# hackmad/pbrt-v3-rs

Hardware: AMD Instinct MI355X
Metric: Mrays/s (higher is better)
Workload: dtype f32

## Files before the change

### include/pbrt_hip.h

```cpp
#ifndef PBRT_HIP_H
#define PBRT_HIP_H

#include <stddef.h>
#include <stdint.h>

#ifdef __cplusplus
extern "C" {
#endif

typedef struct PbrtHipScene PbrtHipScene;

enum {
    PBRT_HIP_OK = 0,
    PBRT_HIP_ERR_INVALID_ARG = -1,
    PBRT_HIP_ERR_STATE = -2,
    PBRT_HIP_ERR_DEVICE = -3,
    PBRT_HIP_ERR_NO_DEVICE = -4,
    PBRT_HIP_ERR_UNSUPPORTED = -5,
    PBRT_HIP_ERR_OOM = -6
};

typedef struct PbrtHipRay {
    float o[3];
    float t_max;
// ... 89 lines not shown
int pbrt_hip_add_texture_checkerboard3d(PbrtHipScene*, uint32_t tex1, uint32_t tex2, const float m[16], uint32_t* out_texture);
enum { PBRT_HIP_PARAM_KD = 0, PBRT_HIP_PARAM_KS = 1, PBRT_HIP_PARAM_KR = 2, PBRT_HIP_PARAM_KT = 3, PBRT_HIP_PARAM_OPACITY = 4, PBRT_HIP_PARAM_AMOUNT = 5, PBRT_HIP_PARAM_ETA = 6,
       PBRT_HIP_PARAM_K = 7, PBRT_HIP_PARAM_REFLECT = 8, PBRT_HIP_PARAM_TRANSMIT = 9 };
int pbrt_hip_set_material_texture(PbrtHipScene*, uint32_t material, int param, uint32_t texture);
int pbrt_hip_set_material_float_texture(PbrtHipScene*, uint32_t material, int fparam, uint32_t texture);
int pbrt_hip_set_material_bump(PbrtHipScene*, uint32_t material, uint32_t texture);
int pbrt_hip_add_material_matte_tex(PbrtHipScene*, uint32_t kd_texture, float sigma_degrees, uint32_t* out_material);
int pbrt_hip_texture_eval_batch(PbrtHipScene*, uint32_t texture, uint64_t n, const float* contexts , float* out_rgb );
int pbrt_hip_texture_eval_batch_nodiff(PbrtHipScene*, uint32_t texture, uint64_t n, const float* contexts , float* out_rgb );
int pbrt_hip_mipmap_levels(PbrtHipScene*, uint32_t mipmap, int* out_levels, int* out_width_height );
int pbrt_hip_mipmap_level_texels(PbrtHipScene*, uint32_t mipmap, int level, float* out_rgb);


int pbrt_hip_add_light_infinite(PbrtHipScene*, const float L_rgb[3], const float light_to_world[16],
                                const float world_to_light[16]);
int pbrt_hip_add_light_infinite_map(PbrtHipScene*, const float L[3], int width, int height, const float* rgb, const float light_to_world[16], const float world_to_light[16]);
int pbrt_hip_add_light_projection(PbrtHipScene*, const float I_rgb[3], const float light_to_world[16], const float world_to_light[16], float fov_deg,
                                  int width, int height, const float* rgb);
int pbrt_hip_add_light_goniometric(PbrtHipScene*, const float I_rgb[3], const float light_to_world[16], const float world_to_light[16],
                                   int width, int height, const float* rgb);
int pbrt_hip_add_light_distant(PbrtHipScene*, const float L_rgb[3], const float w_light_world[3]);
int pbrt_hip_add_light_point(PbrtHipScene*, const float I_rgb[3], const float p_world[3]);
int pbrt_hip_add_light_spot(PbrtHipScene*, const float I_rgb[3], const float light_to_world[16], const float world_to_light[16],
                            float cos_total_width, float cos_falloff_start);
int pbrt_hip_add_light_diffuse_area(PbrtHipScene*, const float L_rgb[3], int two_sided, uint32_t n_tris,
                                    uint32_t* out_first_id);

int pbrt_hip_set_camera_perspective(PbrtHipScene*, const float raster_to_camera[16], const float camera_to_world[16],
                                    float lens_radius, float focal_distance, float shutter_open, float shutter_close);
int pbrt_hip_set_camera_orthographic(PbrtHipScene*, const float raster_to_camera[16], const float camera_to_world[16],
                                     float lens_radius, float focal_distance, float shutter_open, float shutter_close);
int pbrt_hip_set_camera_environment(PbrtHipScene*, const float camera_to_world[16], int xres, int yres, float shutter_open, float shutter_close);

int pbrt_hip_set_film(PbrtHipScene*, int xres, int yres, const int cropped_pixel_bounds[4],
                      const float filter_radius[2], const float filter_table_16x16[256], float scale,
                      float max_sample_luminance);

int pbrt_hip_set_sampler(PbrtHipScene*, int kind, uint32_t samples_per_pixel, const int sample_bounds[4],
                         int sample_at_pixel_center);

int pbrt_hip_set_sobol_tables(PbrtHipScene*, const uint32_t* sobol_matrices32, size_t n32,
                              const uint64_t* vdc_matrices, const uint64_t* vdc_matrices_inv, size_t n_vdc_each);

int pbrt_hip_build_accel(PbrtHipScene*, int split_method, int max_prims_in_node);

int pbrt_hip_build_accel_device(PbrtHipScene*, int split_method, int max_prims_in_node);

int pbrt_hip_world_bound(const PbrtHipScene*, float out_bounds[6]);

int pbrt_hip_accel_stats(const PbrtHipScene*, uint64_t out[8]);
int pbrt_hip_accel_copy(PbrtHipScene*, void* out_nodes, uint64_t node_capacity, void* out_leaf_records, uint64_t record_capacity);


int pbrt_hip_intersect_batch(PbrtHipScene*, const PbrtHipRay* rays, PbrtHipHit* hits, uint64_t n);
int pbrt_hip_occluded_batch(PbrtHipScene*, const PbrtHipRay* rays, uint8_t* out_occluded, uint64_t n);

int pbrt_hip_intersect_batch_device(PbrtHipScene*, const void* d_rays, void* d_hits, uint64_t n, float* kernel_ms);
int pbrt_hip_occluded_batch_device(PbrtHipScene*, const void* d_rays, void* d_occluded, uint64_t n, float* kernel_ms);

int pbrt_hip_set_traversal_counting(PbrtHipScene*, int on);
int pbrt_hip_get_traversal_counts(PbrtHipScene*, uint64_t out[8]);

int pbrt_hip_render_path(PbrtHipScene*, int max_depth, float rr_threshold, int light_strategy,
                         const int pixel_bounds[4], int tile_size, int tile_part, int tile_parts,
                         float* out_xyz, float* out_weight, PbrtHipStats* out_stats);

int pbrt_hip_render_whitted(PbrtHipScene*, int max_depth, const int pixel_bounds[4], int tile_size, int tile_part, int tile_parts,
                            float* out_xyz, float* out_weight, PbrtHipStats* out_stats);

int pbrt_hip_set_sample_record_budget(PbrtHipScene*, uint64_t bytes);
int pbrt_hip_get_render_footprint(PbrtHipScene*, uint64_t out[8]);

int pbrt_hip_tile_buffer_floats(PbrtHipScene*, int tile_size, int tile_part, int tile_parts, uint64_t* out_floats);
int pbrt_hip_render_path_tiles_device(PbrtHipScene*, int max_depth, float rr_threshold, int light_strategy,
                                      const int pixel_bounds[4], int tile_size, int tile_part, int tile_parts,
                                      void* d_tile_buffer, PbrtHipStats* out_stats);
int pbrt_hip_merge_tiles_device(PbrtHipScene*, int tile_size, int tile_parts, const void* const* d_tile_buffers,
                                float* out_xyz, float* out_weight);

int pbrt_hip_film_to_rgb(const PbrtHipScene*, const float* xyz, const float* weight, float* out_rgb);

int pbrt_hip_generate_camera_rays(PbrtHipScene*, const int pixel_bounds[4], uint32_t sample_index,
                                  PbrtHipRay* out_rays, float* out_pfilm_xy);

#ifdef __cplusplus
}
#endif
#endif
```

### pbrt-v3-rs_amd/csrc/api.hip

```cpp
#include "host_math.h"
#include "scene_host.h"
#include "traverse.h"
#include "texture.h"
#include <algorithm>
#include <cstdio>
#include <cstdlib>
#include <mutex>

static std::string g_last_error;
static std::mutex g_err_mu;

namespace phost {

int set_err(PbrtHipScene* s, int code, const std::string& msg) {
    if (s) s->err = msg;
    else { std::lock_guard<std::mutex> g(g_err_mu); g_last_error = msg; }
    return code;
}
int hip_fail(PbrtHipScene* s, hipError_t e, const char* what) {
    std::string m = std::string(what) + ": " + hipGetErrorString(e);
    (void)hipGetLastError();
    return set_err(s, e == hipErrorOutOfMemory ? PBRT_HIP_ERR_OOM : PBRT_HIP_ERR_DEVICE, m);
}
int ensure_buf(PbrtHipScene* s, DevBuf& b, size_t bytes) {
    if (b.bytes >= bytes && b.p) return PBRT_HIP_OK;
    if (b.p) { PH_CHECK(s, hipFree(b.p)); b.p = nullptr; b.bytes = 0; }
    if (bytes == 0) bytes = 16;
    PH_CHECK(s, hipMalloc(&b.p, bytes));
    b.bytes = bytes;
    if (bytes <= 4096) PH_CHECK(s, hipMemset(b.p, 0, bytes));
    return PBRT_HIP_OK;
}

template <class T> static int upload_vec(PbrtHipScene* s, const std::vector<T>& v, const T** out) {
    *out = nullptr;
    if (v.empty()) return PBRT_HIP_OK;
    void* d = nullptr;
    PH_CHECK(s, hipMalloc(&d, v.size() * sizeof(T)));
    s->owned.push_back(d);
    PH_CHECK(s, hipMemcpyAsync(d, v.data(), v.size() * sizeof(T), hipMemcpyHostToDevice, s->stream));
    *out = reinterpret_cast<const T*>(d);
    return PBRT_HIP_OK;
}

void free_tree_dev(PbrtHipScene* s) {
    if (s->tree_dev_nodes) (void)hipFree(s->tree_dev_nodes);
    if (s->tree_dev_tris) (void)hipFree(s->tree_dev_tris);
    s->tree_dev_nodes = s->tree_dev_tris = nullptr; s->tree_dev_n_tris = 0;
}

static void free_owned(PbrtHipScene* s) {
    for (void* p : s->owned) (void)hipFree(p);
    s->owned.clear();
    s->uploaded = false;
    s->light_strategy_uploaded = -1;
}

static hm::HaltonTables& halton_tables() {
    static hm::HaltonTables t;
    static std::once_flag once;
    std::call_once(once, []() { t.build(); });
    return t;
}

__global__ void patch_inst_records_kernel(TriRec* tris, uint32_t n_top, const InstRec* inst, float* extra) {
    const uint32_t i = blockIdx.x * blockDim.x + threadIdx.x;
    if (i >= n_top) return;
    uint32_t f = tris[i].flags & ~PH_TRI_NEXT_INST;
    if (!(f & PH_TRI_LAST) && i + 1u < n_top && (tris[i + 1u].flags & PH_TRI_INSTANCE)) f |= PH_TRI_NEXT_INST;
    if (f & PH_TRI_INSTANCE) {
        const InstRec& I = inst[tris[i].prim];
        const bool general = !(I.w2i[12] == 0.0f && I.w2i[13] == 0.0f && I.w2i[14] == 0.0f && I.w2i[15] == 1.0f);
        for (int k = 0; k < 3; k++) { tris[i].p0[k] = I.lo[k]; tris[i].p1[k] = I.hi[k]; }
        tris[i].p2[0] = __uint_as_float(I.root_ref); tris[i].p2[1] = __uint_as_float(I.flags | (general ? PH_INST_GENERAL : 0u)); tris[i].p2[2] = 0.0f;
        for (int k = 0; k < 12; k++) extra[12 * (size_t)i + k] = I.w2i[k];
    }
    tris[i].flags = f;
}
__global__ void patch_leaf_refs_kernel(Node64* nodes, uint32_t n_nodes, const TriRec* tris, uint32_t n_top) {
    const uint32_t i = blockIdx.x * blockDim.x + threadIdx.x;
    if (i >= n_nodes) return;
    uint32_t c[2] = {nodes[i].c0, nodes[i].c1};
    for (int k = 0; k < 2; k++)
        if ((c[k] & PH_LEAF_BIT) && c[k] < PH_NEED_POP) {
            const uint32_t t = c[k] & ~(PH_LEAF_BIT | PH_LEAF_INST_HINT);
            c[k] = PH_LEAF_BIT | t | ((t < n_top && (tris[t].flags & PH_TRI_INSTANCE)) ? PH_LEAF_INST_HINT : 0u);
        }
    nodes[i].c0 = c[0]; nodes[i].c1 = c[1];
}

int upload_scene(PbrtHipScene* s) {
    if (s->uploaded) return PBRT_HIP_OK;
    free_owned(s);
    DeviceScene& d = s->ds;
    std::memset(&d, 0, sizeof(d));
    int rc;
    if (s->tree_dev_tris) { d.nodes = reinterpret_cast<const Node64*>(s->tree_dev_nodes); d.tris = reinterpret_cast<const TriRec*>(s->tree_dev_tris); }
    else {
        if ((rc = upload_vec(s, s->bvh.nodes, &d.nodes))) return rc;
        if ((rc = upload_vec(s, s->bvh.tris, &d.tris))) return rc;
    }
    d.root_ref = s->bvh.root_ref;
    d.n_tris = (uint32_t)(s->idx.size() / 3);
    for (int k = 0; k < 3; k++) { d.root_lo[k] = s->bvh.root_lo[k]; d.root_hi[k] = s->bvh.root_hi[k]; d.world_center[k] = s->world_center[k]; }
    d.world_radius = s->world_radius;
    if ((rc = upload_vec(s, s->P, &d.P))) return rc;
    if (s->any_n && (rc = upload_vec(s, s->N, &d.N))) return rc;
    if (s->any_s && (rc = upload_vec(s, s->S, &d.S))) return rc;
    if (s->any_uv && (rc = upload_vec(s, s->UV, &d.UV))) return rc;
    if ((rc = upload_vec(s, s->idx, &d.idx))) return rc;
    if ((rc = upload_vec(s, s->tri_mesh, &d.tri_mesh))) return rc;
    if ((rc = upload_vec(s, s->tri_flags, &d.tri_flags))) return rc;
    if (s->emission_only.empty()) { if ((rc = upload_vec(s, s->meshes, &d.meshes))) return rc; }
    else {
        std::vector<MeshRec> meshes(s->meshes);
        for (MeshRec& m : meshes) if (m.first_light <= -2) m.first_light = (int32_t)(s->lights.size() + (size_t)(-2 - m.first_light));
        if ((rc = upload_vec(s, meshes, &d.meshes))) return rc;
    }
    {
        for (MaterialRec& m : s->materials) {
            uint32_t cols = m.amount_tex1 ? 1u : 0u; bool hdr = m.bump_tex1 != 0u || m.sigma_tex1 != 0u;
            for (uint32_t k = 0; k < m.n_lobes; k++) {
                s->lobes[m.lobe_base + k].slot0 = cols;
                const LobeRec& l = s->lobes[m.lobe_base + k];
                if (l.has_pre == PH_PRE_RT) { cols += 1u; hdr = true; }
                else cols += (l.r_tex1 || (l.has_pre == PH_PRE_OPACITY && l.kind != PH_LK_SPEC_T) ? 1u : 0u) + (l.t_tex1 || (l.has_pre == PH_PRE_OPACITY && l.kind == PH_LK_SPEC_T) || l.has_pre == PH_PRE_PASSTHROUGH ? 1u : 0u) +
                        (l.eta_tex1 ? 1u : 0u) + (l.k_tex1 ? 1u : 0u);
                if (l.sigma_tex1 || l.ax_tex1 || l.ay_tex1 || l.alt || l.has_pre == PH_PRE_RAW_TEST) hdr = true;
            }
            if (m.sigma_tex1 || hdr) cols = std::max(cols, 2u);
            if (m.index_tex1) cols = std::max(cols, 3u);
            if (m.rt_mode) hdr = true;
            m.tex_cols = std::min<uint32_t>(cols, PH_HIT_COLS); m.tex_hdr = hdr ? 1u : 0u;
        }
        s->alpha_lean = s->alpha_textures;
        for (const MeshRec& m : s->meshes)
            for (uint32_t t1 : {m.alpha_tex1, m.shadow_alpha_tex1})
                if (t1)
                    for (const TexOp& op : s->textures[t1 - 1u].prog)
                        if (!(op.op == PH_TOP_CONST || op.op == PH_TOP_MUL || op.op == PH_TOP_MIX || (op.op == PH_TOP_IMAGE && op.mapping == 0u))) s->alpha_lean = false;
        s->simple_textures = true;
        for (const PbrtHipScene::TextureHost& t : s->textures)
            for (const TexOp& op : t.prog)
                if (!(op.op == PH_TOP_CONST || op.op == PH_TOP_MUL || op.op == PH_TOP_MIX || (op.op == PH_TOP_IMAGE && op.mapping == 0u))) s->simple_textures = false;
    }
    if ((rc = upload_vec(s, s->materials, &d.materials))) return rc;
    if ((rc = upload_vec(s, s->lobes, &d.lobes))) return rc;
    {
        const uint32_t kMaxTex = 500u, kMaxPlain = 500u;
        std::vector<uint16_t> key(std::max<size_t>(s->materials.size(), 1), 0);
        uint32_t n_tex = 0, n_plain = 0;
        for (const MaterialRec& m : s->materials) if (!m.none && (m.textured || m.bump_tex1)) n_tex++;
        const uint32_t T = std::min(n_tex, kMaxTex);
        uint32_t jt = 0, jp = 0;
        for (size_t i = 0; i < s->materials.size(); i++) {
            const MaterialRec& m = s->materials[i];
            if (!m.none && (m.textured || m.bump_tex1)) key[i] = (uint16_t)std::min(jt++, kMaxTex - 1u);
            else { key[i] = (uint16_t)(T + std::min(jp++, kMaxPlain - 1u)); n_plain++; }
        }
        const uint32_t U = std::min(n_plain, kMaxPlain);
        if ((rc = upload_vec(s, key, &d.mat_key))) return rc;
        d.ms_tex_keys = T; d.ms_key_emit = T + U; d.ms_key_idle = T + U + 1u;
    }
    if (!s->textures.empty() || !s->mipmaps.empty()) {
        std::vector<TexRec> recs; std::vector<TexOp> ops;
        for (const PbrtHipScene::TextureHost& t : s->textures) {
            recs.push_back(TexRec{(uint32_t)ops.size(), (uint32_t)t.prog.size()});
            ops.insert(ops.end(), t.prog.begin(), t.prog.end());
        }
        std::vector<float> lut(PH_EWA_LUT_SIZE);
        for (int i = 0; i < PH_EWA_LUT_SIZE; i++) {
            const float r2 = (float)i / (float)(PH_EWA_LUT_SIZE - 1);
            lut[(size_t)i] = std::exp(-2.0f * r2) - std::exp(-2.0f);
        }
        if ((rc = upload_vec(s, recs, &d.textures))) return rc;
        if ((rc = upload_vec(s, ops, &d.tex_ops))) return rc;
        if ((rc = upload_vec(s, s->mipmaps, &d.mipmaps))) return rc;
        if ((rc = upload_vec(s, s->texels, &d.texels))) return rc;
        if ((rc = upload_vec(s, lut, &d.ewa_lut))) return rc;
    }
    if (s->emission_only.empty()) { if ((rc = upload_vec(s, s->lights, &d.lights))) return rc; }
    else {
        std::vector<LightRec> all(s->lights);
        all.insert(all.end(), s->emission_only.begin(), s->emission_only.end());
        if ((rc = upload_vec(s, all, &d.lights))) return rc;
    }
    if ((rc = upload_vec(s, s->light_dist, &d.light_dist))) return rc;
    d.n_lights = (uint32_t)s->lights.size();
    if ((rc = upload_vec(s, s->infinite_lights, &d.infinite_lights))) return rc;
    d.n_infinite = (uint32_t)s->infinite_lights.size();
    if ((rc = upload_vec(s, s->inst_recs, &d.instances))) return rc;
    if ((rc = upload_vec(s, s->quadrics, &d.quadrics))) return rc;
    d.n_instances = (uint32_t)s->inst_recs.size();
    if (!s->inst_recs.empty() && !s->top_items.empty() && d.tris) {
        const uint32_t n_top = (uint32_t)s->top_items.size();
        const uint32_t n_nodes = (uint32_t)(s->tree_dev_tris ? s->bvh.interior_nodes : s->bvh.nodes.size());
        void* extra = nullptr;
        PH_CHECK(s, hipMalloc(&extra, (size_t)n_top * 48)); s->owned.push_back(extra);
        hipLaunchKernelGGL(patch_inst_records_kernel, dim3((n_top + 255u) / 256u), dim3(256), 0, s->stream, const_cast<TriRec*>(d.tris), n_top, d.instances, static_cast<float*>(extra));
        if (n_nodes) hipLaunchKernelGGL(patch_leaf_refs_kernel, dim3((n_nodes + 255u) / 256u), dim3(256), 0, s->stream, const_cast<Node64*>(d.nodes), n_nodes, d.tris, n_top);
        PH_CHECK(s, hipGetLastError());
        d.inst_extra = static_cast<const float*>(extra);
    }
    hm::HaltonTables& ht = halton_tables();
    if ((rc = upload_vec(s, ht.perms, &d.halton_perms))) return rc;
    if ((rc = upload_vec(s, ht.primes, &d.primes))) return rc;
    if ((rc = upload_vec(s, ht.prime_sums, &d.prime_sums))) return rc;
    if ((rc = upload_vec(s, ht.magic, &d.prime_magic))) return rc;
    if ((rc = upload_vec(s, s->sobol32, &d.sobol32))) return rc;
    if ((rc = upload_vec(s, s->vdc, &d.vdc))) return rc;
    if ((rc = upload_vec(s, s->vdc_inv, &d.vdc_inv))) return rc;
    {
        void* dself = nullptr;
        PH_CHECK(s, hipMalloc(&dself, sizeof(DeviceScene)));
        s->owned.push_back(dself);
        d.self = reinterpret_cast<const DeviceScene*>(dself);
        PH_CHECK(s, hipMemcpyAsync(dself, &d, sizeof(DeviceScene), hipMemcpyHostToDevice, s->stream));
    }
    PH_CHECK(s, hipStreamSynchronize(s->stream));
    s->uploaded = true;
    return PBRT_HIP_OK;
}

int upload_light_distribution(PbrtHipScene* s, int light_strategy) {
    const size_t n = s->lights.size();
    int strat = (n == 1) ? 0 : light_strategy;
    if (s->light_strategy_uploaded == strat) return PBRT_HIP_OK;
    std::vector<float> f(n, 1.0f), cdf;
    float func_int = 0.0f;
    if (strat == 1) {
        const float wr = s->world_radius;
        for (size_t i = 0; i < n; i++) {
            const LightRec& l = s->lights[i];
            float p[3];
            for (int c = 0; c < 3; c++) {
                switch (l.type) {
                case PH_L_INFINITE: {
                    if (l.map_mip1) { float t[3]; hmip_lookup_triangle(s, s->mipmaps[l.map_mip1 - 1u], 0.5f, 0.5f, 0.5f, t); p[c] = hm::kPi * wr * wr * t[c]; break; }
                    float tx = l.L[c];
                    float v = tx * (1.0f - 0.0f) * (1.0f - 0.0f) + tx * (1.0f - 0.0f) * 0.0f + tx * 0.0f * (1.0f - 0.0f) + tx * 0.0f * 0.0f;
                    p[c] = hm::kPi * wr * wr * v;
                    break;
                }
                case PH_L_DISTANT: p[c] = l.L[c] * hm::kPi * wr * wr; break;
                case PH_L_POINT: p[c] = (hm::kPi * 4.0f) * l.L[c]; break;
                case PH_L_PROJECTION: case PH_L_GONIO: {
                    float t[3] = {1.0f, 1.0f, 1.0f};
                    if (l.map_mip1) hmip_lookup_triangle(s, s->mipmaps[l.map_mip1 - 1u], 0.5f, 0.5f, 0.5f, t);
                    p[c] = l.type == PH_L_PROJECTION ? t[c] * l.L[c] * (2.0f * hm::kPi) * (1.0f - l.cos_total_width) : (hm::kPi * 4.0f) * l.L[c] * t[c];
                    break;
                }
                case PH_L_SPOT: p[c] = l.L[c] * (2.0f * hm::kPi) * (1.0f - 0.5f * (l.cos_falloff_start + l.cos_total_width)); break;
                default: p[c] = (l.two_sided ? 2.0f : 1.0f) * l.L[c] * l.area * hm::kPi; break;
                }
            }
            f[i] = 0.212671f * p[0] + 0.715160f * p[1] + 0.072169f * p[2];
        }
    }
    if (n) hm::distribution1d(f, cdf, func_int);
    int rc;
    if ((rc = ensure_buf(s, s->d_ld_func, std::max<size_t>(n, 1) * 4))) return rc;
    if ((rc = ensure_buf(s, s->d_ld_cdf, (n + 1) * 4))) return rc;
    if (n) {
        PH_CHECK(s, hipMemcpy(s->d_ld_func.p, f.data(), n * 4, hipMemcpyHostToDevice));
        PH_CHECK(s, hipMemcpy(s->d_ld_cdf.p, cdf.data(), (n + 1) * 4, hipMemcpyHostToDevice));
    }
    s->ds.ld_func = (const float*)s->d_ld_func.p; s->ds.ld_cdf = (const float*)s->d_ld_cdf.p; s->ds.ld_func_int = func_int;
    s->light_strategy_uploaded = strat;
    return PBRT_HIP_OK;
}

int ensure_traversal_workspace(PbrtHipScene* s) {
    if (!s->trav_blocks) {
        hipDeviceProp_t prop;
        PH_CHECK(s, hipGetDeviceProperties(&prop, s->device));
        int per_cu = 0;
        PH_CHECK(s, hipOccupancyMaxActiveBlocksPerMultiprocessor(&per_cu, ph::traverse_kernel<ph::ShapeFlat, ph::TRAV_MIXED>, PH_TRAV_BLOCK, 0));
        per_cu = std::max(std::min(per_cu, ph::ShapeFlat::wpe), 1);
        s->trav_blocks = (uint32_t)(prop.multiProcessorCount * per_cu);
    }
    const uint32_t total_threads = s->trav_blocks * PH_TRAV_BLOCK;
    int rc;
    if ((rc = ensure_buf(s, s->d_counter, 64))) return rc;
    if ((rc = ensure_buf(s, s->d_error, 64))) return rc;
    if ((rc = ensure_buf(s, s->d_counts, 64 + 36 * 8))) return rc;
    const bool inst = !s->inst_recs.empty();
    if ((rc = ensure_buf(s, s->d_spill, (size_t)(ph::trav_stack_cap(inst) - ph::TravShapes::spill_lds_depth(inst)) * total_threads * sizeof(uint2)))) return rc;
    return PBRT_HIP_OK;
}

template <class Shape>
static void launch_traverse_shape(PbrtHipScene* s, int mode, uint32_t blocks, const ph::TravParams& p) {
    const dim3 g(blocks), b(PH_TRAV_BLOCK);
    if (mode == ph::TRAV_MIXED) hipLaunchKernelGGL((ph::traverse_kernel<Shape, ph::TRAV_MIXED>), g, b, 0, s->stream, s->ds, p);
    else if (mode == ph::TRAV_ANY) hipLaunchKernelGGL((ph::traverse_kernel<Shape, ph::TRAV_ANY>), g, b, 0, s->stream, s->ds, p);
    else hipLaunchKernelGGL((ph::traverse_kernel<Shape, ph::TRAV_CLOSEST>), g, b, 0, s->stream, s->ds, p);
}
template <class... S>
static void dispatch_traverse_shape(ph::ShapeTable<S...>, int shape, PbrtHipScene* s, int mode, uint32_t blocks, const ph::TravParams& p) {
    static constexpr void (*launchers[])(PbrtHipScene*, int, uint32_t, const ph::TravParams&) = {&launch_traverse_shape<S>...};
    launchers[shape](s, mode, blocks, p);
}

// ... 868 lines not shown
    if (out_first_id) *out_first_id = (uint32_t)s->lights.size();
    for (uint32_t i = 0; i < n_tris; i++) {
        LightRec l{}; l.type = PH_L_AREA; l.two_sided = two_sided ? 1 : 0; l.prim = 0xFFFFFFFFu;
        for (int c = 0; c < 3; c++) l.L[c] = L[c];
        s->lights.push_back(l);
    }
    s->uploaded = false;
    return PBRT_HIP_OK;
    });
}

int pbrt_hip_set_camera_perspective(PbrtHipScene* s, const float r2c[16], const float c2w[16], float lens_radius, float focal_distance,
                                    float shutter_open, float shutter_close) {
    return ph_guard(s, "pbrt_hip_set_camera_perspective", [&]() -> int {
    if (!s || !r2c || !c2w) return set_err(s, PBRT_HIP_ERR_INVALID_ARG, "set_camera_perspective: null argument");
    std::memcpy(s->cam.r2c, r2c, 64); std::memcpy(s->cam.c2w, c2w, 64);
    s->cam.lens_radius = lens_radius; s->cam.focal_distance = focal_distance;
    s->cam.shutter_open = shutter_open; s->cam.shutter_close = shutter_close;
    {
        auto pt = [&](float x, float y, float out[3]) {
            const float* m = r2c;
            const float xp = m[0] * x + m[1] * y + m[2] * 0.0f + m[3], yp = m[4] * x + m[5] * y + m[6] * 0.0f + m[7];
            const float zp = m[8] * x + m[9] * y + m[10] * 0.0f + m[11], wp = m[12] * x + m[13] * y + m[14] * 0.0f + m[15];
            if (wp == 1.0f) { out[0] = xp; out[1] = yp; out[2] = zp; }
            else { const float inv = 1.0f / wp; out[0] = inv * xp; out[1] = inv * yp; out[2] = inv * zp; }
        };
        float p0[3], px[3], py[3];
        pt(0.0f, 0.0f, p0); pt(1.0f, 0.0f, px); pt(0.0f, 1.0f, py);
        for (int k = 0; k < 3; k++) { s->cam.dx_camera[k] = px[k] - p0[k]; s->cam.dy_camera[k] = py[k] - p0[k]; }
    }
    s->cam.kind = PH_CAM_PERSPECTIVE;
    s->have_camera = true;
    return PBRT_HIP_OK;
    });
}
int pbrt_hip_set_camera_orthographic(PbrtHipScene* s, const float r2c[16], const float c2w[16], float lens_radius, float focal_distance,
                                     float shutter_open, float shutter_close) {
    return ph_guard(s, "pbrt_hip_set_camera_orthographic", [&]() -> int {
    const int rc = pbrt_hip_set_camera_perspective(s, r2c, c2w, lens_radius, focal_distance, shutter_open, shutter_close);
    if (rc != PBRT_HIP_OK) return rc;
    const float* m = r2c;
    const float vx[3] = {1.0f, 0.0f, 0.0f}, vy[3] = {0.0f, 1.0f, 0.0f};
    for (int k = 0; k < 3; k++) {
        s->cam.dx_camera[k] = m[4 * k] * vx[0] + m[4 * k + 1] * vx[1] + m[4 * k + 2] * vx[2];
        s->cam.dy_camera[k] = m[4 * k] * vy[0] + m[4 * k + 1] * vy[1] + m[4 * k + 2] * vy[2];
    }
    s->cam.kind = PH_CAM_ORTHOGRAPHIC;
    return PBRT_HIP_OK;
    });
}

int pbrt_hip_set_camera_environment(PbrtHipScene* s, const float c2w[16], int xres, int yres, float shutter_open, float shutter_close) {
    return ph_guard(s, "pbrt_hip_set_camera_environment", [&]() -> int {
    if (!s || !c2w) return set_err(s, PBRT_HIP_ERR_INVALID_ARG, "set_camera_environment: null argument");
    if (xres <= 0 || yres <= 0) return set_err(s, PBRT_HIP_ERR_INVALID_ARG, "set_camera_environment: the film's full resolution must be positive");
    s->cam = CameraRec{};
    for (int k = 0; k < 4; k++) s->cam.r2c[5 * k] = 1.0f;
    std::memcpy(s->cam.c2w, c2w, 64);
    s->cam.focal_distance = 1e6f; s->cam.shutter_open = shutter_open; s->cam.shutter_close = shutter_close;
    s->cam.full_res[0] = (float)xres; s->cam.full_res[1] = (float)yres;
    s->cam.kind = PH_CAM_ENVIRONMENT;
    s->have_camera = true;
    return PBRT_HIP_OK;
    });
}

int pbrt_hip_set_film(PbrtHipScene* s, int xres, int yres, const int crop[4], const float radius[2], const float table[256], float scale,
                      float max_lum) {
    return ph_guard(s, "pbrt_hip_set_film", [&]() -> int {
    if (!s || !crop || !radius || !table) return set_err(s, PBRT_HIP_ERR_INVALID_ARG, "set_film: null argument");
    if (!(radius[0] > 0.0f) || !(radius[1] > 0.0f)) return set_err(s, PBRT_HIP_ERR_INVALID_ARG, "set_film: filter radius must be positive");
    FilmRec& f = s->film;
    f.xres = xres; f.yres = yres;
    for (int i = 0; i < 4; i++) f.crop[i] = crop[i];
    f.radius[0] = radius[0]; f.radius[1] = radius[1];
    f.inv_radius[0] = 1.0f / radius[0]; f.inv_radius[1] = 1.0f / radius[1];
    f.scale = scale; f.max_lum = max_lum;
    std::memcpy(f.table, table, sizeof(f.table));
    s->have_film = true;
    return PBRT_HIP_OK;
    });
}

static void ext_gcd(uint64_t a, uint64_t b, int64_t& x, int64_t& y) {
    if (b == 0) { x = 1; y = 0; return; }
    int64_t d = (int64_t)(a / b), xp, yp;
    ext_gcd(b, a % b, xp, yp);
    x = yp; y = xp - (d * yp);
}
static uint64_t mult_inverse(int64_t a, int64_t n) {
    int64_t x, y;
    ext_gcd((uint64_t)a, (uint64_t)n, x, y);
    int64_t r = x - (x / n) * n;
    return (uint64_t)(r < 0 ? r + n : r);
}

int pbrt_hip_set_sampler(PbrtHipScene* s, int kind, uint32_t spp, const int sb[4], int at_center) {
    return ph_guard(s, "pbrt_hip_set_sampler", [&]() -> int {
    if (!s || !sb) return set_err(s, PBRT_HIP_ERR_INVALID_ARG, "set_sampler: null argument");
    if (kind != 0 && kind != 1) return set_err(s, PBRT_HIP_ERR_UNSUPPORTED, "set_sampler: only halton (0) and sobol (1) are GPU-friendly (SURVEY §8a-S)");
    if (spp == 0) return set_err(s, PBRT_HIP_ERR_INVALID_ARG, "set_sampler: spp must be > 0");
    SamplerRec& r = s->sampler;
    std::memset(&r, 0, sizeof(r));
    r.kind = kind; r.spp = spp; r.at_center = at_center ? 1 : 0;
    for (int i = 0; i < 4; i++) r.bounds[i] = sb[i];
    if (kind == 0) {
        int res[2] = {sb[2] - sb[0], sb[3] - sb[1]};
        for (int i = 0; i < 2; i++) {
            uint64_t base = i == 0 ? 2 : 3, scale = 1, e = 0;
            while ((int)scale < std::min(res[i], 128)) { scale *= base; e++; }
            r.base_scales[i] = (uint32_t)scale; r.base_exponents[i] = (uint32_t)e;
        }
        r.sample_stride = r.base_scales[0] * r.base_scales[1];
        r.mult_inverse[0] = (uint32_t)mult_inverse(r.base_scales[1], r.base_scales[0]);
        r.mult_inverse[1] = (uint32_t)mult_inverse(r.base_scales[0], r.base_scales[1]);
        if (((uint64_t)spp + 1) * r.sample_stride >= (1ull << 32))
            return set_err(s, PBRT_HIP_ERR_UNSUPPORTED, "set_sampler: halton index exceeds 32 bits at this spp/resolution");
    } else {
        auto pow2_up = [](uint32_t v) { v--; v |= v >> 1; v |= v >> 2; v |= v >> 4; v |= v >> 8; v |= v >> 16; return v + 1; };
        if (spp & (spp - 1)) r.spp = pow2_up(spp);
        int ext = std::max(sb[2] - sb[0], sb[3] - sb[1]);
        r.resolution = (int)pow2_up((uint32_t)std::max(ext, 1));
        int lg = 0; for (uint32_t v = (uint32_t)r.resolution; v >>= 1;) lg++;
        r.log2_resolution = lg;
    }
    s->have_sampler = true;
    return PBRT_HIP_OK;
    });
}

int pbrt_hip_set_sobol_tables(PbrtHipScene* s, const uint32_t* m32, size_t n32, const uint64_t* vdc, const uint64_t* vdc_inv, size_t n_each) {
    return ph_guard(s, "pbrt_hip_set_sobol_tables", [&]() -> int {
    if (!s || !m32 || !vdc || !vdc_inv) return set_err(s, PBRT_HIP_ERR_INVALID_ARG, "set_sobol_tables: null argument");
    if (n32 == 0 || n32 % 52 || n_each % 52) return set_err(s, PBRT_HIP_ERR_INVALID_ARG, "set_sobol_tables: table lengths must be non-zero multiples of 52");
    s->sobol32.assign(m32, m32 + n32); s->vdc.assign(vdc, vdc + n_each); s->vdc_inv.assign(vdc_inv, vdc_inv + n_each);
    s->uploaded = false;
    return PBRT_HIP_OK;
    });
}

int pbrt_hip_build_accel(PbrtHipScene* s, int split_method, int max_prims_in_node) {
    return ph_guard(s, "pbrt_hip_build_accel", [&]() -> int {
    if (!s) return PBRT_HIP_ERR_INVALID_ARG;
    if (split_method == 2) return set_err(s, PBRT_HIP_ERR_UNSUPPORTED, "build_accel: splitmethod 'middle' panics in the reference (quirk B6, sah.rs:67-76)");
    if (!s->quadrics.empty()) {
        if (s->build_on_device) return set_err(s, PBRT_HIP_ERR_UNSUPPORTED, "build_accel_device: a scene with quadric shapes is built on the host (pbrt_hip_build_accel)");
        if (!s->objects.empty() || !s->instances.empty()) return set_err(s, PBRT_HIP_ERR_UNSUPPORTED, "build_accel: quadric shapes together with object definitions or instances are not supported");
        s->prim_quadric.resize(s->idx.size() / 3, 0u);
    }
    for (size_t i = 0; i < s->lights.size(); i++)
        if (s->lights[i].type == PH_L_AREA && s->lights[i].prim == 0xFFFFFFFFu)
            return set_err(s, PBRT_HIP_ERR_STATE, "build_accel: area light " + std::to_string(i) + " was never attached to a mesh (pbrt_hip_add_mesh first_area_light_id)");
    {
        std::vector<uint64_t> sigs;
        for (MaterialRec& m : s->materials) {
            uint64_t sig = 1;
            for (uint32_t k = 0; k < m.n_lobes; k++) sig = sig * 8 + (s->lobes[m.lobe_base + k].kind + 1);
            size_t c = 0;
            while (c < sigs.size() && sigs[c] != sig) c++;
            if (c == sigs.size()) sigs.push_back(sig);
            m.sort_class = (uint32_t)std::min<size_t>(c, 6);
            if (m.none) m.sort_class = 7u;
        }
    }
    if (s->tree_dev_tris) { PH_CHECK(s, hipSetDevice(s->device)); free_tree_dev(s); }
    std::vector<uint32_t> build_flags(s->tri_flags);
    for (size_t t = 0; t < build_flags.size(); t++) {
        const uint32_t mat = s->meshes[s->tri_mesh[t]].material;
        build_flags[t] |= (s->materials[mat].sort_class << PH_TRI_CLASS_SHIFT) | (std::min<uint32_t>(mat, 0xFFFu) << PH_TRI_MAT_SHIFT);
    }
    phost::BuildInput in;
    in.P = s->P.data(); in.idx = s->idx.data(); in.n_tris = s->idx.size() / 3; in.tri_flags = build_flags.data(); in.tri_mesh = s->tri_mesh.data();
    if (!s->quadrics.empty()) { in.prim_quadric = s->prim_quadric.data(); in.quad_bounds = s->quadric_bounds.data(); }
    auto fail = [&](int brc) {
        if (brc == -2) return set_err(s, PBRT_HIP_ERR_INVALID_ARG, "build_accel: the reference's HLBVH build asserts on this input (hlbvh.rs:338/356/418)");
        return set_err(s, PBRT_HIP_ERR_INVALID_ARG, "build_accel: bad arguments");
    };
    s->inst_recs.clear();
    if (s->objects.empty()) {
        int brc;
        if (s->build_on_device) {
            PH_CHECK(s, hipSetDevice(s->device));
            std::string e;
            if (split_method == 1) brc = phost::build_hlbvh_device(in, max_prims_in_node, s->stream, s->bvh, e);
            else {
                brc = phost::build_sah_device(in, max_prims_in_node, s->stream, s->bvh, e, &s->tree_dev_nodes, &s->tree_dev_tris);
                if (brc == 0 && s->tree_dev_tris) s->tree_dev_n_tris = in.n_tris;
            }
            if (brc == -1) return set_err(s, PBRT_HIP_ERR_DEVICE, "build_accel_device: " + e);
        } else brc = phost::build_bvh(in, split_method, max_prims_in_node, 0, s->bvh);
        if (brc != 0) return fail(brc);
    } else {
        if (s->open_object >= 0) return set_err(s, PBRT_HIP_ERR_STATE, "build_accel: an object definition is still open (missing ObjectEnd)");
        std::vector<uint32_t> tri0(s->objects.size()), tri1(s->objects.size()), inst_object(s->instances.size());
        std::vector<float> inst_i2w(16 * s->instances.size());
        for (size_t k = 0; k < s->objects.size(); k++) { tri0[k] = s->objects[k].tri0; tri1[k] = s->objects[k].tri1; }
        for (size_t k = 0; k < s->instances.size(); k++) { inst_object[k] = s->instances[k].object; std::memcpy(&inst_i2w[16 * k], s->instances[k].i2w, 64); }
        const phost::InstancedScene isc{tri0.data(), tri1.data(), tri0.size(), inst_object.data(), inst_i2w.data(), inst_object.size(), s->top_items.data(), s->top_items.size()};
// ... 204 lines not shown
```

### pbrt-v3-rs_amd/csrc/host_math.h

```cpp
#pragma once
#include <cmath>
#include <cstdint>
#include <cstring>
#include <vector>

namespace hm {

constexpr float kPi = 3.14159265358979323846f;
constexpr float kInf = __builtin_huge_valf();

inline float fabs_p(float n) { return n < 0.0f ? -n : n; }
inline float clampf(float x, float lo, float hi) { return x < lo ? lo : (x > hi ? hi : x); }
inline float to_radians(float d) { return d * (kPi / 180.0f); }

struct V3 { float x, y, z; };
inline V3 sub(V3 a, V3 b) { return {a.x - b.x, a.y - b.y, a.z - b.z}; }
inline V3 add(V3 a, V3 b) { return {a.x + b.x, a.y + b.y, a.z + b.z}; }
inline V3 mulf(V3 a, float f) { return {a.x * f, a.y * f, a.z * f}; }
inline V3 divf(V3 a, float f) { float inv = 1.0f / f; return {inv * a.x, inv * a.y, inv * a.z}; }
inline V3 cross(V3 a, V3 b) { return {(a.y * b.z) - (a.z * b.y), (a.z * b.x) - (a.x * b.z), (a.x * b.y) - (a.y * b.x)}; }
inline float len2(V3 a) { return a.x * a.x + a.y * a.y + a.z * a.z; }
inline float len(V3 a) { return std::sqrt(len2(a)); }
inline V3 normalize(V3 a) { return divf(a, len(a)); }
inline void coordinate_system(V3 v1, V3& v2, V3& v3) {
    if (std::fabs(v1.x) > std::fabs(v1.y)) v2 = divf({-v1.z, 0.0f, v1.x}, std::sqrt(v1.x * v1.x + v1.z * v1.z));
    else v2 = divf({0.0f, v1.z, -v1.y}, std::sqrt(v1.y * v1.y + v1.z * v1.z));
    v3 = cross(v1, v2);
}
inline V3 ld(const float* p) { return {p[0], p[1], p[2]}; }

struct Pcg32 {
    uint64_t state = 0x853c49e6748fea9bULL, inc = 0xda3e39cb94b95bdbULL;
    uint32_t next() {
        uint64_t old = state;
        state = old * 0x5851f42d4c957f2dULL + inc;
        uint32_t xs = (uint32_t)(((old >> 18) ^ old) >> 27), rot = (uint32_t)(old >> 59);
        return (xs >> rot) | (xs << ((~rot + 1) & 31));
    }
    uint32_t bounded(uint32_t lo, uint32_t hi) {
        uint32_t b = hi - lo, threshold = (~b + 1) % b;
        for (;;) { uint32_t r = next(); if (r >= threshold) return lo + r % b; }
    }
};

inline float radical_inverse(uint32_t base, uint64_t a) {
    if (base == 2) {
        uint64_t n = a;
        n = ((n >> 1) & 0x5555555555555555ULL) | ((n & 0x5555555555555555ULL) << 1);
        n = ((n >> 2) & 0x3333333333333333ULL) | ((n & 0x3333333333333333ULL) << 2);
        n = ((n >> 4) & 0x0f0f0f0f0f0f0f0fULL) | ((n & 0x0f0f0f0f0f0f0f0fULL) << 4);
        n = ((n >> 8) & 0x00ff00ff00ff00ffULL) | ((n & 0x00ff00ff00ff00ffULL) << 8);
        n = ((n >> 16) & 0x0000ffff0000ffffULL) | ((n & 0x0000ffff0000ffffULL) << 16);
        n = (n >> 32) | (n << 32);
        return (float)n * 0x1.0p-64f;
    }
    const float inv_base = 1.0f / (float)base;
    uint64_t reversed = 0; float inv_base_n = 1.0f;
    while (a != 0) {
        const uint64_t next = a / base, digit = a - next * base;
        reversed = reversed * base + digit;
        inv_base_n *= inv_base;
        a = next;
    }
    const float v = (float)reversed * inv_base_n;
    return v < 0x1.fffffep-1f ? v : 0x1.fffffep-1f;
}

struct HaltonTables {
    std::vector<uint32_t> primes, prime_sums;
    std::vector<uint16_t> perms;
    std::vector<uint64_t> magic;
    void build() {
        primes.clear(); prime_sums.clear();
        for (uint32_t c = 2; primes.size() < 1000; c++) {
            bool is_p = true;
            for (uint32_t q : primes) { if (q * q > c) break; if (c % q == 0) { is_p = false; break; } }
            if (is_p) primes.push_back(c);
        }
        uint32_t total = 0;
        magic.clear();
        for (uint32_t p : primes) { prime_sums.push_back(total); total += p; magic.push_back((uint64_t)(((unsigned __int128)1 << 64) / p) + 1); }
        perms.assign(total, 0);
        Pcg32 rng; size_t at = 0;
        for (uint32_t p : primes) {
            for (uint32_t j = 0; j < p; j++) perms[at + j] = (uint16_t)j;
            for (uint32_t j = 0; j < p; j++) {
                uint32_t other = j + rng.bounded(0, p - j);
                uint16_t t = perms[at + j]; perms[at + j] = perms[at + other]; perms[at + other] = t;
            }
            at += p;
        }
    }
};

inline void distribution1d(const std::vector<float>& f, std::vector<float>& cdf, float& func_int) {
    size_t n = f.size();
    cdf.assign(n + 1, 0.0f);
    for (size_t i = 1; i < n + 1; i++) cdf[i] = cdf[i - 1] + f[i - 1] / (float)n;
    func_int = cdf[n];
    if (func_int == 0.0f) for (size_t i = 1; i < n + 1; i++) cdf[i] = (float)i / (float)n;
    else for (size_t i = 1; i < n + 1; i++) cdf[i] /= func_int;
}

struct M4 { float m[4][4]; };
inline M4 m4_identity() { M4 r; for (int i = 0; i < 4; i++) for (int j = 0; j < 4; j++) r.m[i][j] = i == j ? 1.0f : 0.0f; return r; }
inline M4 m4_mul(const M4& a, const M4& b) {
    M4 r;
    for (int i = 0; i < 4; i++)
        for (int j = 0; j < 4; j++)
            r.m[i][j] = a.m[i][0] * b.m[0][j] + a.m[i][1] * b.m[1][j] + a.m[i][2] * b.m[2][j] + a.m[i][3] * b.m[3][j];
    return r;
}
inline M4 m4_transpose(const M4& a) { M4 r; for (int i = 0; i < 4; i++) for (int j = 0; j < 4; j++) r.m[i][j] = a.m[j][i]; return r; }
M4 m4_inverse(const M4& a);

}
```

### pbrt-v3-rs_amd/csrc/pt_device.h

```cpp
#pragma once
#include "dmath.h"
#include "scene_types.h"
#include "traverse.h"

namespace ph {

struct f2 { float x, y; };
PH_DEV f2 mk2(float x, float y) { f2 r; r.x = x; r.y = y; return r; }

PH_DEV float radical_inverse_2(uint64_t a) {
    uint64_t r = ((uint64_t)__brev((uint32_t)a) << 32) | (uint64_t)__brev((uint32_t)(a >> 32));
    return __ull2float_rn(r) * 0x1.0p-64f;
}
PH_DEV float radical_inverse_base(uint32_t base, uint32_t a) {
    const float inv_base = ph_div(1.0f, (float)base);
    uint64_t reversed = 0;
    float inv_base_n = 1.0f;
    while (a != 0) {
        uint32_t next = a / base, digit = a - next * base;
        reversed = reversed * base + digit;
        inv_base_n *= inv_base;
        a = next;
    }
    return pminf(__ull2float_rn(reversed) * inv_base_n, kOneMinusEps);
}
PH_DEV float scrambled_radical_inverse(uint32_t base, uint64_t magic, uint32_t a, const uint16_t* __restrict__ perm) {
    const float inv_base = ph_div(1.0f, (float)base);
    uint64_t reversed = 0;
    float inv_base_n = 1.0f;
    while (a != 0) {
        uint32_t next = (uint32_t)__umul64hi((uint64_t)a, magic), digit = a - next * base;
        reversed = reversed * base + perm[digit];
        inv_base_n *= inv_base;
        a = next;
    }
    return pminf(inv_base_n * (__ull2float_rn(reversed) + ph_div(inv_base * (float)perm[0], 1.0f - inv_base)), kOneMinusEps);
}
PH_DEV uint32_t inverse_radical_inverse(uint32_t base, uint32_t inverse, uint32_t n_digits) {
    uint32_t index = 0;
    for (uint32_t i = 0; i < n_digits; i++) { uint32_t digit = inverse % base; inverse /= base; index = index * base + digit; }
    return index;
}
PH_DEV int rem_i(int a, int b) { int r = a - (a / b) * b; return r < 0 ? r + b : r; }

PH_DEV uint32_t halton_pixel_offset(const SamplerRec& sp, int px, int py) {
    uint64_t off = 0;
    if (sp.sample_stride > 1) {
        const int pm[2] = {rem_i(px, 128), rem_i(py, 128)};
        for (int i = 0; i < 2; i++) {
            uint64_t dim_offset = inverse_radical_inverse(i == 0 ? 2u : 3u, (uint32_t)pm[i], sp.base_exponents[i]);
            off += dim_offset * (uint64_t)(sp.sample_stride / sp.base_scales[i]) * (uint64_t)sp.mult_inverse[i];
        }
        off %= sp.sample_stride;
    }
    return (uint32_t)off;
}
#define PH_LDS_DIMS 54
#define PH_LDS_PERMS 6081
struct HaltonLds {
    uint8_t perms[PH_LDS_PERMS + 2];
    uint32_t primes[PH_LDS_DIMS], sums[PH_LDS_DIMS];
    uint64_t magic[PH_LDS_DIMS];
};
PH_DEV void halton_lds_fill(HaltonLds* l, const DeviceScene& sc) {
    for (uint32_t i = threadIdx.x; i < PH_LDS_PERMS; i += blockDim.x) l->perms[i] = (uint8_t)sc.halton_perms[i];
    for (uint32_t i = threadIdx.x; i < PH_LDS_DIMS; i += blockDim.x) { l->primes[i] = sc.primes[i]; l->sums[i] = sc.prime_sums[i]; l->magic[i] = sc.prime_magic[i]; }
}
PH_DEV float scrambled_radical_inverse_lds(const HaltonLds* l, uint32_t dim, uint32_t a) {
    const uint32_t base = l->primes[dim];
    const uint64_t magic = l->magic[dim];
    const uint8_t* perm = l->perms + l->sums[dim];
    const float inv_base = ph_div(1.0f, (float)base);
    uint64_t reversed = 0;
    float inv_base_n = 1.0f;
    while (a != 0) {
        uint32_t next = (uint32_t)__umul64hi((uint64_t)a, magic), digit = a - next * base;
        reversed = reversed * base + perm[digit];
        inv_base_n *= inv_base;
        a = next;
    }
    return pminf(inv_base_n * (__ull2float_rn(reversed) + ph_div(inv_base * (float)perm[0], 1.0f - inv_base)), kOneMinusEps);
}
PH_DEV float halton_sample(const DeviceScene& sc, const SamplerRec& sp, uint32_t index, uint32_t dim, const HaltonLds* lds = nullptr) {
    if (sp.at_center && (dim == 0 || dim == 1)) return 0.5f;
    if (dim == 0) return radical_inverse_2((uint64_t)(index >> sp.base_exponents[0]));
    if (dim == 1) return radical_inverse_base(3u, index / sp.base_scales[1]);
    if (lds && dim < PH_LDS_DIMS) return scrambled_radical_inverse_lds(lds, dim, index);
    return scrambled_radical_inverse(sc.primes[dim], sc.prime_magic[dim], index, sc.halton_perms + sc.prime_sums[dim]);
}

PH_DEV uint64_t sobol_interval_to_index(const DeviceScene& sc, uint32_t m, uint64_t frame, int px, int py) {
    if (m == 0) return 0;
    const uint32_t m2 = m << 1;
    uint64_t index = frame << m2;
    uint64_t delta = 0;
    for (int c = 0; frame != 0; frame >>= 1, c++)
        if (frame & 1) delta ^= sc.vdc[(size_t)(m - 1) * 52 + c];
    uint64_t b = ((((uint64_t)(uint32_t)px) << m) | ((uint64_t)(uint32_t)py)) ^ delta;
    for (int c = 0; b != 0; b >>= 1, c++)
        if (b & 1) index ^= sc.vdc_inv[(size_t)(m - 1) * 52 + c];
    return index;
}
PH_DEV float sobol_sample(const DeviceScene& sc, const SamplerRec& sp, uint64_t a, uint32_t dim, int px, int py) {
    uint32_t v = 0;
    for (size_t i = (size_t)dim * 52; a != 0; a >>= 1, i++)
        if (a & 1) v ^= sc.sobol32[i];
    float s = pminf((float)v * 0x1.0p-32f, kOneMinusEps);
    if (dim == 0 || dim == 1) {
        s = s * (float)sp.resolution + (float)sp.bounds[dim];
        s = pclampf(s - (float)(dim == 0 ? px : py), 0.0f, kOneMinusEps);
    }
    return s;
}

struct SamplerCursor {
    uint64_t index;
    uint32_t dim;
    int px, py;
    const HaltonLds* lds;
};
PH_DEV float sampler_dim(const DeviceScene& sc, const SamplerRec& sp, const SamplerCursor& c, uint32_t dim) {
    return sp.kind == 0 ? halton_sample(sc, sp, (uint32_t)c.index, dim, c.lds) : sobol_sample(sc, sp, c.index, dim, c.px, c.py);
}
PH_DEV float get_1d(const DeviceScene& sc, const SamplerRec& sp, SamplerCursor& c) {
    float p = sampler_dim(sc, sp, c, c.dim);
    c.dim += 1;
    return p;
}
PH_DEV f2 get_2d(const DeviceScene& sc, const SamplerRec& sp, SamplerCursor& c) {
    if (c.dim + 1 >= 5 && c.dim < 5) c.dim = 5;
    f2 p = mk2(sampler_dim(sc, sp, c, c.dim), sampler_dim(sc, sp, c, c.dim + 1));
    c.dim += 2;
    return p;
}

PH_DEV f2 concentric_sample_disk(f2 u) {
    f2 uo = mk2(2.0f * u.x - 1.0f, 2.0f * u.y - 1.0f);
    if (uo.x == 0.0f && uo.y == 0.0f) return mk2(0.0f, 0.0f);
    float r, theta;
    if (pabs(uo.x) > pabs(uo.y)) { r = uo.x; theta = kPiOver4 * ph_div(uo.y, uo.x); }
    else { r = uo.y; theta = kPiOver2 - kPiOver4 * ph_div(uo.x, uo.y); }
    float sn, cs;
    d_sincos(theta, sn, cs);
    return mk2(r * cs, r * sn);
}
PH_DEV f3 cosine_sample_hemisphere(f2 u) {
    f2 d = concentric_sample_disk(u);
    float z = ph_sqrt(pmaxf(0.0f, 1.0f - d.x * d.x - d.y * d.y));
    return mk3(d.x, d.y, z);
}
PH_DEV f2 uniform_sample_triangle(f2 u) { float su0 = ph_sqrt(u.x); return mk2(1.0f - su0, u.y * su0); }
PH_DEV float power_heuristic1(float fp, float gp) {
    float f = 1.0f * fp, g = 1.0f * gp;
    return ph_div(f * f, f * f + g * g);
}
PH_DEV uint32_t find_interval_cdf(const float* cdf, uint32_t size, float u) {
    uint32_t first = 0, len = size;
    while (len > 0) {
        uint32_t half = len >> 1, middle = first + half;
        if (cdf[middle] <= u) { first = middle + 1; len -= half + 1; }
        else len = half;
    }
    if (first == 0) return 0;
    uint32_t v = first - 1, hi = size - 2;
    return v > hi ? hi : v;
}

__device__ __noinline__ void environment_camera_dir(float px, float py, float xres, float yres, f3* out) {
    const float theta = ph_div(kPi * py, yres), phi = ph_div(kTwoPi * px, xres);
    const float st = d_sin(theta);
    *out = mk3(st * d_cos(phi), d_cos(theta), st * d_sin(phi));
}
PH_DEV void generate_camera_ray(const CameraRec& cam, f2 p_film, float time_s, f2 lens_s, RayIn& out) {
    const float* m = cam.r2c;
    float xp = m[0] * p_film.x + m[1] * p_film.y + m[2] * 0.0f + m[3];
    float yp = m[4] * p_film.x + m[5] * p_film.y + m[6] * 0.0f + m[7];
    float zp = m[8] * p_film.x + m[9] * p_film.y + m[10] * 0.0f + m[11];
    float wp = m[12] * p_film.x + m[13] * p_film.y + m[14] * 0.0f + m[15];
    f3 p_camera = (wp == 1.0f) ? mk3(xp, yp, zp) : mk3(xp, yp, zp) / wp;
    f3 o = mk3(0.0f, 0.0f, 0.0f), d = normalize(p_camera);
    if (cam.kind == PH_CAM_ORTHOGRAPHIC) { o = p_camera; d = mk3(0.0f, 0.0f, 1.0f); }
    if (cam.kind == PH_CAM_ENVIRONMENT) environment_camera_dir(p_film.x, p_film.y, cam.full_res[0], cam.full_res[1], &d);
    const float time = (1.0f - time_s) * cam.shutter_open + time_s * cam.shutter_close;
    if (cam.lens_radius > 0.0f) {
        f2 cd = concentric_sample_disk(lens_s);
        f2 p_lens = mk2(cam.lens_radius * cd.x, cam.lens_radius * cd.y);
        float ft = ph_div(cam.focal_distance, d.z);
        f3 p_focus = o + d * ft;
        o = mk3(p_lens.x, p_lens.y, 0.0f);
        d = normalize(p_focus - o);
    }
    const float* c = cam.c2w;
    float ox = (c[0] * o.x + c[1] * o.y) + (c[2] * o.z + c[3]);
    float oy = (c[4] * o.x + c[5] * o.y) + (c[6] * o.z + c[7]);
    float oz = (c[8] * o.x + c[9] * o.y) + (c[10] * o.z + c[11]);
    float ow = (c[12] * o.x + c[13] * o.y) + (c[14] * o.z + c[15]);
    float xs = pabs(c[0] * o.x) + pabs(c[1] * o.y) + pabs(c[2] * o.z) + pabs(c[3]);
    float ys = pabs(c[4] * o.x) + pabs(c[5] * o.y) + pabs(c[6] * o.z) + pabs(c[7]);
    float zs = pabs(c[8] * o.x) + pabs(c[9] * o.y) + pabs(c[10] * o.z) + pabs(c[11]);
    f3 o_err = kGamma3 * mk3(xs, ys, zs);
    f3 ow3 = (ow == 1.0f) ? mk3(ox, oy, oz) : mk3(ox, oy, oz) / ow;
    f3 dw = mk3(c[0] * d.x + c[1] * d.y + c[2] * d.z, c[4] * d.x + c[5] * d.y + c[6] * d.z, c[8] * d.x + c[9] * d.y + c[10] * d.z);
    float l2 = length_squared(dw), t_max = kInf;
    if (l2 > 0.0f) {
        float dt = ph_div(dot(vabs(dw), o_err), l2);
// ... 393 lines not shown
```

### pbrt-v3-rs_amd/csrc/scene_host.h

```cpp
#pragma once
#include "../../include/pbrt_hip.h"
#include "band_plan.h"
#include "bvh_build.h"
#include "guard.h"
#include "scene_types.h"
#include <hip/hip_runtime.h>
namespace ph { struct TravParams; }
#include <string>
#include <vector>

struct DevBuf {
    void* p = nullptr;
    size_t bytes = 0;
};

struct SceneHostState {
    std::vector<float> P, N, S, UV;
    bool any_n = false, any_s = false, any_uv = false;
    std::vector<uint32_t> idx, tri_mesh, tri_flags;
    std::vector<MeshRec> meshes;
    std::vector<QuadricRec> quadrics;
    std::vector<float> quadric_bounds;
    std::vector<uint32_t> prim_quadric;
    std::vector<MaterialRec> materials;
    std::vector<LobeRec> lobes;
    struct TextureHost { std::vector<TexOp> prog; int stack_need = 1; };
    std::vector<TextureHost> textures;
    std::vector<MipRec> mipmaps;
    std::vector<Texel> texels;
    struct MaterialParams { int lobe[4] = {-1, -1, -1, -1}; int field[4] = {0, 0, 0, 0}; int lobe2[4] = {-1, -1, -1, -1}; int field2[4] = {0, 0, 0, 0}; bool has_pre = false; float pre[3] = {1, 1, 1}; int rough_lobe = -1, rough_lobe2 = -1; bool rough_remap = false;
                            int made_as = 0;   float raw_k[4][3] = {{0, 0, 0}, {0, 0, 0}, {0, 0, 0}, {0, 0, 0}}; float raw_eta = 1.5f, raw_ur = 0, raw_vr = 0;
                            bool raw_remap = false, rebuilt = false; int mix_n1 = 0; };
    std::vector<MaterialParams> material_params;
    bool alpha_textures = false;
    bool alpha_lean = false;
    bool bump_materials = false;
    bool textured_materials = false;
    bool has_none_material = false;
    bool general_materials = false;
    bool simple_textures = false;
    std::vector<LightRec> lights;
    uint32_t sphere_lights = 0;
    std::vector<LightRec> emission_only;
    std::vector<uint32_t> infinite_lights;
    std::vector<float> light_dist;
    struct ObjectHost { uint32_t tri0 = 0, tri1 = 0; };
    struct InstanceHost { uint32_t object; float i2w[16], w2i[16]; };
    std::vector<ObjectHost> objects;
    std::vector<InstanceHost> instances;
    std::vector<uint32_t> top_items;
    int open_object = -1;
    std::vector<InstRec> inst_recs;
    CameraRec cam{};
    FilmRec film{};
    SamplerRec sampler{};
    bool have_camera = false, have_film = false, have_sampler = false, built = false;
    std::vector<uint32_t> sobol32;
    std::vector<uint64_t> vdc, vdc_inv;

    phost::BuildOutput bvh;
    float world_center[3] = {0, 0, 0}, world_radius = 1.0f;
};

struct MultiDevice;

struct PbrtHipScene : SceneHostState {
    int device = 0;
    hipStream_t stream = nullptr;
    std::string err;
    bool build_on_device = false;
    MultiDevice* multi = nullptr;

    DeviceScene ds{};
    std::vector<void*> owned;
    void* tree_dev_nodes = nullptr; void* tree_dev_tris = nullptr; size_t tree_dev_n_tris = 0;
    bool uploaded = false;
    int light_strategy_uploaded = -1;
    DevBuf d_ld_func, d_ld_cdf;

    DevBuf d_counter, d_spill, d_error, d_rays_tmp, d_out_tmp;
    uint32_t trav_blocks = 0;
    bool count_traversal = false;
    DevBuf d_counts;
    hipEvent_t ev0 = nullptr, ev1 = nullptr;

    struct Wavefront* wf = nullptr;
    struct WhittedWorkspace* wh = nullptr;

    uint64_t record_budget = 0;
    uint64_t footprint[8] = {0, 0, 0, 0, 0, 0, 0, 0};
};

namespace phost {
int set_err(PbrtHipScene* s, int code, const std::string& msg);
int hip_fail(PbrtHipScene* s, hipError_t e, const char* what);
int ensure_buf(PbrtHipScene* s, DevBuf& b, size_t bytes);
int upload_scene(PbrtHipScene* s);
void projection_light_setup(float fov_deg, float aspect, float out_proj[16], float out_screen[4], float* out_cos_total_width);
void hmip_lookup_triangle(const PbrtHipScene* s, const MipRec& m, float u, float v, float width, float out[3]);
int upload_light_distribution(PbrtHipScene* s, int light_strategy);
int launch_traverse(PbrtHipScene* s, bool anyhit, const void* d_rays, void* d_out, uint32_t n, float* kernel_ms);
void launch_traverse_kernel(PbrtHipScene* s, int mode, uint32_t blocks, const ph::TravParams& p);
int ensure_traversal_workspace(PbrtHipScene* s);
void free_wavefront(PbrtHipScene* s);
int build_hlbvh_device(const BuildInput& in, int max_prims_in_node, hipStream_t stream, BuildOutput& out, std::string& err, const ForestSpec* forest = nullptr,
                       std::vector<ForestTreeOut>* trees_out = nullptr);
int build_sah_device(const BuildInput& in, int max_prims_in_node, hipStream_t stream, BuildOutput& out, std::string& err, void** keep_nodes = nullptr, void** keep_tris = nullptr,
                     const ForestSpec* forest = nullptr, std::vector<ForestTreeOut>* trees_out = nullptr);
void free_tree_dev(PbrtHipScene* s);
int uber_rebuild_for_opacity(PbrtHipScene* s, uint32_t material);
int glass_rebuild_for_roughness(PbrtHipScene* s, uint32_t material);
int translucent_rebuild_rt(PbrtHipScene* s, uint32_t material);
#define PH_MAX_TILE_PARTS 64
int check_render_args(PbrtHipScene* s, int max_depth, int light_strategy, const int* pixel_bounds, int tile_size, int part, int parts);
size_t tile_buffer_floats_for(const PbrtHipScene* s, int tile_size, int part, int parts);
int render_tiles(PbrtHipScene* s, int max_depth, float rr_threshold, int light_strategy, const int pixel_bounds[4], int tile_size, int part, int parts, void* d_tile_buffer,
                 PbrtHipStats* out_stats);
int merge_tiles(PbrtHipScene* s, int tile_size, int parts, const void* const* d_bufs, float* out_xyz, float* out_weight);
DevBuf& tile_buffer_of(PbrtHipScene* s);
int merge_own_tiles(PbrtHipScene* s, int tile_size, int tile_part, int tile_parts, float* out_xyz, float* out_weight);
struct SampleRecords { uint32_t n_px; const int2* px_xy; float4* rec_L; float* rec_py; uint8_t* px_rounded; SampleBand band; uint32_t band_px; std::vector<SampleBand> bands; };
int samples_begin(PbrtHipScene* s, int tile_size, int part, int parts, SampleRecords* out);
int samples_plan_bands(PbrtHipScene* s, SampleRecords* out, size_t chunk_held, size_t chunk_per_path);
int samples_alloc(PbrtHipScene* s, SampleRecords* out);
int samples_band(PbrtHipScene* s, const SampleRecords& r, size_t band, SampleRecords* out);
int samples_to_tiles(PbrtHipScene* s, const SampleRecords& r, void* d_tile_buffer);
size_t path_chunk_bytes_per_path(bool general_materials, bool textured_materials);
void free_whitted(PbrtHipScene* s);
size_t whitted_chunk_bytes_per_sample(uint32_t n_frames);
int spatial_voxels_touched(PbrtHipScene* s, std::vector<uint8_t>& touched, uint64_t* count);
int render_path_multi(PbrtHipScene* s, int max_depth, float rr_threshold, int light_strategy, const int pixel_bounds[4], int tile_size, int tile_part, int tile_parts,
                      float* out_xyz, float* out_weight, PbrtHipStats* out_stats);
void free_multi(PbrtHipScene* s);
}

#define PH_CHECK(s, call)                                              \
    do {                                                               \
        hipError_t e__ = (call);                                       \
        if (e__ != hipSuccess) return phost::hip_fail((s), e__, #call); \
    } while (0)
```

### pbrt-v3-rs_amd/csrc/scene_types.h

```cpp
#pragma once
#include <stdint.h>

#define PH_LEAF_BIT 0x80000000u
#define PH_INVALID_REF 0xFFFFFFFFu
#define PH_NEED_POP 0xFFFFFFFEu
#define PH_LEAF_INST_HINT 0x40000000u
struct alignas(64) Node64 {
    float x0[2], y0[2], z0[2];
    float x1[2], y1[2], z1[2];
    uint32_t c0, c1;
    uint32_t axis;
    uint32_t pad;
};

#define PH_TRI_LAST 1u
#define PH_TRI_BOGUS 2u
#define PH_TRI_ALPHA0 4u
#define PH_TRI_SALPHA0 8u
#define PH_TRI_CLASS_SHIFT 8
#define PH_TRI_MAT_SHIFT 11
#define PH_TRI_KEY_MASK 0x7FFFu
#define PH_TRI_ALPHATEX 32u
#define PH_TRI_NEXT_INST 64u
#define PH_TRI_INSTANCE 16u
// ... 85 lines not shown
    uint32_t refl_tex1, trans_tex1;
    float refl_c[3], trans_c[3];
    uint32_t index_tex1;
    uint32_t tex_cols;
    uint32_t tex_hdr;
};
#define PH_HIT_COLS 6
struct TexOut { float ns[3]; uint32_t bumped; float dpdu_s[3]; uint32_t lambert; float col[PH_HIT_COLS][4]; };
#define PH_HIT_LOBES 8

enum { PH_TOP_CONST = 0, PH_TOP_IMAGE = 1, PH_TOP_MUL = 2, PH_TOP_MIX = 3, PH_TOP_CHECKER = 4 , PH_TOP_UV = 5,
       PH_TOP_BILERP = 6 , PH_TOP_DOTS = 7 , PH_TOP_FBM = 8, PH_TOP_WRINKLED = 9, PH_TOP_WINDY = 10, PH_TOP_MARBLE = 11,
       PH_TOP_CHECKER3D = 12  };
#define PH_TEX_STACK 6
struct TexOp {
    uint32_t op;
    uint32_t mip;
    float c[3];
    float su, sv, du, dv;
    uint32_t octaves;
    float omega, scale, variation;
    float m[16];
    uint32_t mapping;
    uint32_t pad_[3];
};
struct TexRec { uint32_t first_op, n_ops; };
struct Texel { float r, g, b, pad; };
#define PH_MIP_MAX_LEVELS 16
struct MipRec {
    uint32_t n_levels, filtering , wrap , is_float;
    float max_anisotropy;
    uint32_t pad[3];
    uint32_t level_off[PH_MIP_MAX_LEVELS];
    uint32_t level_w[PH_MIP_MAX_LEVELS], level_h[PH_MIP_MAX_LEVELS];
};
#define PH_EWA_LUT_SIZE 128

enum { PH_L_INFINITE = 0, PH_L_DISTANT = 1, PH_L_POINT = 2, PH_L_AREA = 3, PH_L_SPOT = 4, PH_L_PROJECTION = 5, PH_L_GONIO = 6 };
struct LightRec {
    int32_t type;
    int32_t two_sided;
    uint32_t prim;
    float area;
    float L[3];
    uint32_t map_mip1;
    float v[3];
    uint32_t dist_off;
    float l2w[12];
    float w2l[12];
    float cond_func[4], cond_cdf[6], cond_int[2];
    float marg_func[2], marg_cdf[3], marg_int;
    float cos_total_width, cos_falloff_start;
    uint32_t dw, dh;
    float proj[16];
    float screen[4];
};

enum { PH_CAM_PERSPECTIVE = 0, PH_CAM_ORTHOGRAPHIC = 1, PH_CAM_ENVIRONMENT = 2 };
struct CameraRec {
    float r2c[16];
    float c2w[16];
    float lens_radius, focal_distance, shutter_open, shutter_close;
    float dx_camera[3], dy_camera[3];
    uint32_t kind; float pad[1];
    float full_res[2];
};

struct FilmRec {
    int32_t xres, yres;
    int32_t crop[4];
    float radius[2], inv_radius[2];
    float scale, max_lum;
    float table[256];
};

struct SamplerRec {
    int32_t kind;
    uint32_t spp;
    int32_t bounds[4];
    int32_t at_center;
    uint32_t base_scales[2], base_exponents[2], sample_stride;
    uint32_t mult_inverse[2];
    int32_t resolution, log2_resolution;
};

struct DeviceScene {
    const Node64* nodes;
    const TriRec* tris;
    uint32_t root_ref;
    uint32_t n_tris;
    float root_lo[3], root_hi[3];
    float world_center[3], world_radius;
    const float* P;
    const float* N;
    const float* S;
    const float* UV;
    const uint32_t* idx;
    const uint32_t* tri_mesh;
    const uint32_t* tri_flags;
    const MeshRec* meshes;
    const MaterialRec* materials;
    const LobeRec* lobes;
    const TexRec* textures;
    const TexOp* tex_ops;
    const MipRec* mipmaps;
    const Texel* texels;
    const float* ewa_lut;
    const float* light_dist;
    const DeviceScene* self;
    const LightRec* lights;
    uint32_t n_lights;
    const uint32_t* infinite_lights;
    uint32_t n_infinite;
    const uint16_t* mat_key;
    uint32_t ms_tex_keys, ms_key_emit, ms_key_idle;
    const InstRec* instances;
    const float* inst_extra;
    uint32_t n_instances;
    const float* ld_func;
    const float* ld_cdf;
    float ld_func_int;
    const uint16_t* halton_perms;
    const uint32_t* primes;
    const uint32_t* prime_sums;
    const uint64_t* prime_magic;
    const uint32_t* sobol32;
    const uint64_t* vdc;
    const uint64_t* vdc_inv;
    const QuadricRec* quadrics;
};
```

### pbrt-v3-rs_amd/csrc/wavefront.hip

```cpp
#define PH_OUTLINE_MATH 1
#include "host_math.h"
#include "pt_device.h"
#include "scene_host.h"
#include "spatial.h"
#include "bsdf_general.h"
#include "texture.h"
#include "raysort.h"
#include "phase_clock.h"
#include "matsort.h"
#include "wf_device.h"
#include "chunk_plan.h"
#include <algorithm>
#include <cstdlib>

namespace ph {

enum : uint32_t { F_EXT = 1u, F_PSH = 2u, F_PMIS = 4u, F_SPEC = 8u, F_NODIFF = 16u };

struct IterCounters {
    uint32_t n_cl, n_sh, n_live, head_cl, head_sh, pad[3];
};
struct DevStats { unsigned long long camera_rays, paths_total, paths_zero; };

struct TileInfo {
// ... 271 lines not shown
                    if (!w.occ[idx4.z]) est = est + mks(A4.x, A4.y, A4.z);
                }
                if (flags & F_PMIS) {
                    const float4 F4 = w.s_f2[it & 1][prev];
                    const uint32_t light_num = __float_as_uint(F4.w);
                    const RayIn mr = load_ray(rays_in + idx4.y);
                    const float4* hp = reinterpret_cast<const float4*>(w.hits_cl + idx4.y);
                    const float4 h0 = hp[0];
                    const uint32_t hprim = __float_as_uint(h0.y);
                    const f3 wi = mk3(mr.dx, mr.dy, mr.dz);
                    spec li2 = mks1(0.0f);
                    if (hprim != 0xFFFFFFFFu) {
                        const LightRec& lt = sc.lights[light_num];
                        if (lt.type == PH_L_AREA && lt.prim == hprim) {
                            const float4 h1 = hp[1];
                            MeshRec m;
                            SurfHit lh = make_surface_hit_any(sc, wi, mr.time, __float_as_uint(h1.y), __float_as_uint(h1.z), h0.z, h0.w, h1.x, m);
                            li2 = area_L(lt, lh.n, -wi);
                        }
                    } else li2 = light_le<TEX>(sc, sc.lights[light_num], wi);
                    if (!is_black(li2)) est = est + mks(F4.x, F4.y, F4.z) * li2 * mks1(1.0f) * A4.w / O4.w;
                }
                const spec ldv = mks(O4.x, O4.y, O4.z) * (est / L4.w);
                if (is_black(ldv)) n_paths_zero++;
                L = L + ldv;
                flags &= ~(F_PSH | F_PMIS);
            }
            PHC_END(0);

            if (flags & F_EXT) {
                flags &= ~F_EXT;
                const RayIn ray = load_ray(rays_in + idx4.x);
                const float4* hp = reinterpret_cast<const float4*>(w.hits_cl + idx4.x);
                const float4 h0 = hp[0];
                const uint32_t hprim = __float_as_uint(h0.y);
                const bool found = hprim != 0xFFFFFFFFu;
                const f3 rd = mk3(ray.dx, ray.dy, ray.dz);
                const bool emit = bounces == 0 || (GEN && (flags & F_SPEC));
                if (!found) {
                    if (emit)
                        for (uint32_t k = 0; k < sc.n_infinite; k++) L = L + beta * light_le<TEX>(sc, sc.lights[sc.infinite_lights[k]], rd);
                } else {
                    const float4 h1 = hp[1];
                    MeshRec m;
                    PHC_BEGIN(1);
                    QSurf qs;
                    SurfHit si = QUADRIC ? make_surface_hit_q<QUADRIC>(sc, mk3(ray.ox, ray.oy, ray.oz), rd, ray.time, __float_as_uint(h1.y), __float_as_uint(h1.z), h0.z, h0.w, h1.x, m, &qs)
                                         : make_surface_hit_any(sc, rd, ray.time, __float_as_uint(h1.y), __float_as_uint(h1.z), h0.z, h0.w, h1.x, m);
                    if (emit) {
                        if (m.first_light >= 0) L = L + beta * area_L(sc.lights[(uint32_t)m.first_light + (hprim - m.tri_base)], si.n, -rd);
                        else L = L + beta * mks1(0.0f);
                    }
                    PHC_END(1);
                    bool no_bsdf = sc.materials[m.material].none != 0u;
                    if (TEX && !no_bsdf && sc.materials[m.material].rt_mode) no_bsdf = (w.tex_out[i].bumped & PH_TEXOUT_NULL_BSDF) != 0u;
                    if ((int)bounces < w.max_depth && no_bsdf) {
                        const RayIn re = spawn_ray(si, rd);
                        flags |= F_EXT | F_NODIFF; want_ext = true;
                        stage[0][0][tid] = make_float4(re.ox, re.oy, re.oz, re.t_max);
                        stage[0][1][tid] = make_float4(re.dx, re.dy, re.dz, re.time);
                    } else if ((int)bounces < w.max_depth) {
                        const uint32_t ppix = pid / w.chunk_spp;
                        const int2 xy = w.px_xy[ppix];
                        bool tex_hit = false;
                        if (TEX) {
                            const MaterialRec& mr = sc.materials[m.material];
                            tex_hit = mr.textured != 0u || mr.bump_tex1 != 0u;
                            if (tex_hit && mr.bump_tex1) {
                                const float4* tp = reinterpret_cast<const float4*>(w.tex_out + i);
                                const float4 f0 = tp[0], f1 = tp[1];
                                si.ns = mk3(f0.x, f0.y, f0.z); si.dpdu_s = mk3(f1.x, f1.y, f1.z);
                            }
                        }
                        PHC_BEGIN(2);
                        typename BO::T bsdf = BO::make(sc, si, m.material);
                        if (TEX && tex_hit) {
                            const MaterialRec& mr = sc.materials[m.material];
                            if (mr.textured)
                                BO::apply_textures(bsdf, w.tex_out + i, mr);
                        }
                        PHC_END(2);
                        PHC_BEGIN(3);
                        SamplerCursor cur = cursor_for(sc, w.sp, xy.x, xy.y, w.s0 + (pid - ppix * w.chunk_spp), dim, hl);
#pragma unroll 1
                        for (uint32_t k = 0; k < 8; k++) s_u[k][tid] = sampler_dim(sc, w.sp, cur, dim + k);
                        PHC_END(3);
                        uint32_t c = 0;
                        if (BO::has_non_specular(bsdf)) {
                            n_paths_total++;
                            if (sc.n_lights > 0) {
                                PHC_BEGIN(4);
                                const float sample = s_u[0][tid]; c = 1;
                                const float* ld_func = sc.ld_func; const float* ld_cdf = sc.ld_cdf; float ld_func_int = sc.ld_func_int;
                                if (w.spatial.enabled) {
                                    const int32_t slot = w.spatial.vox_slot[spatial_voxel_of(w.spatial, si.p)];
                                    if (slot >= 0) {
                                        ld_func = w.spatial.pool + (size_t)slot * w.spatial.stride;
                                        ld_cdf = ld_func + sc.n_lights; ld_func_int = ld_cdf[sc.n_lights + 1];
                                    } else ld_func_int = 0.0f;
                                }
                                const uint32_t light_num = (sc.n_lights == 1) ? 0u : find_interval_cdf(ld_cdf, sc.n_lights + 1, sample);
                                pick_pdf = ld_func_int > 0.0f ? ph_div(ld_func[light_num], ld_func_int * (float)sc.n_lights) : 0.0f;
                                PHC_END(4);
                                if (pick_pdf != 0.0f) {
                                    const LightRec& light = sc.lights[light_num];
                                    const f2 u_light = mk2(s_u[1][tid], s_u[2][tid]), u_scatter = mk2(s_u[3][tid], s_u[4][tid]); c = 5;
                                    const bool is_delta = light.type == PH_L_DISTANT || light.type == PH_L_POINT || light.type == PH_L_SPOT || light.type == PH_L_PROJECTION || light.type == PH_L_GONIO;
                                    float w2 = 0.0f, spdf_store = 0.0f;
                                    spec A = mks1(0.0f);
                                    {
                                        PHC_BEGIN(5);
                                        const LiSample ls = light_sample_li<TEX>(sc, light, si, u_light);
                                        PHC_END(5);
                                        PHC_BEGIN(6);
                                        if (ls.valid && ls.pdf > 0.0f && !is_black(ls.value)) {
                                            const spec f = BO::f_ns(bsdf, si.wo, ls.wi) * abs_dot(ls.wi, si.ns);
                                            const float scattering_pdf = BO::pdf_ns(bsdf, si.wo, ls.wi);
                                            if (!is_black(f)) {
                                                const RayIn rs = spawn_ray_to_hit(si, ls.vp, ls.vperr, ls.vn);
                                                stage[2][0][tid] = make_float4(rs.ox, rs.oy, rs.oz, rs.t_max);
                                                stage[2][1][tid] = make_float4(rs.dx, rs.dy, rs.dz, rs.time);
                                                want_sh = true;
                                                if (is_delta) A = f * ls.value / ls.pdf;
                                                else A = f * ls.value * power_heuristic1(ls.pdf, scattering_pdf) / ls.pdf;
                                                flags |= F_PSH;
                                            }
                                        }
                                        PHC_END(6);
                                    }
                                    if (!is_delta) {
                                        PHC_BEGIN(7);
                                        spec f1; float spdf; f3 wi2;
                                        BO::sample_ns(bsdf, si.wo, u_scatter, f1, spdf, wi2);
                                        const spec f = f1 * abs_dot(wi2, si.ns);
                                        if (!is_black(f) && spdf > 0.0f) {
                                            const float lp = light_pdf_li<TEX>(sc, light, si, wi2);
                                            if (lp != 0.0f) {
                                                w2 = power_heuristic1(spdf, lp);
                                                spdf_store = spdf;
                                                const RayIn rm = spawn_ray(si, wi2);
                                                stage[1][0][tid] = make_float4(rm.ox, rm.oy, rm.oz, rm.t_max);
                                                stage[1][1][tid] = make_float4(rm.dx, rm.dy, rm.dz, rm.time);
                                                want_mis = true;
                                                w.s_f2[(it + 1) & 1][i] = make_float4(f.r, f.g, f.b, __uint_as_float(light_num));
                                                flags |= F_PMIS;
                                            }
                                        }
                                        PHC_END(7);
                                    }
                                    if (flags & (F_PSH | F_PMIS)) {
                                        w.s_A[(it + 1) & 1][i] = make_float4(A.r, A.g, A.b, w2);
                                        w.s_bold[(it + 1) & 1][i] = make_float4(beta.r, beta.g, beta.b, spdf_store);
                                    }
                                }
                            }
                            if (!(flags & (F_PSH | F_PMIS))) n_paths_zero++;
                        }
                        PHC_BEGIN(8);
                        const f2 u = mk2(s_u[c][tid], s_u[c + 1][tid]); c += 2;
                        spec f; float pdf; f3 wi; uint32_t stype;
                        BO::sample_all(bsdf, -rd, u, f, pdf, wi, stype);
                        flags &= ~F_SPEC;
                        if (!(is_black(f) || pdf == 0.0f)) {
                            beta = beta * (f * abs_dot(wi, si.ns) / pdf);
                            if (GEN) {
                                if (stype & BX_SPEC) flags |= F_SPEC;
                                if ((stype & BX_SPEC) && (stype & BX_TRANS)) {
                                    const float eta = BO::eta(bsdf);
// ... 137 lines not shown
                    if (r.w != r.w) continue;
                    if ((up_y && pfy != (float)(sy + 1)) || (up_x && r.w != (float)(sx + 1))) continue;
                    const float pfx = r.w;
                    spec l = mks(r.x, r.y, r.z);
                    const float ly = lum_y(l);
                    if (ly > p.film.max_lum) l = l * p.film.max_lum / ly;
                    const float pdx = pfx - 0.5f, pdy = pfy - 0.5f;
                    int p0x = f2i_sat(ceilf(pdx - rx)), p0y = f2i_sat(ceilf(pdy - ry));
                    int p1x = f2i_sat(floorf(pdx + rx)) + 1, p1y = f2i_sat(floorf(pdy + ry)) + 1;
                    p0x = pmaxi(p0x, t.pb[0]); p0y = pmaxi(p0y, t.pb[1]); p1x = pmini(p1x, t.pb[2]); p1y = pmini(p1y, t.pb[3]);
                    if (x < p0x || x >= p1x || y < p0y || y >= p1y) continue;
                    const float fx = pabs(((float)x - pdx) * p.film.inv_radius[0] * 16.0f);
                    const float fy = pabs(((float)y - pdy) * p.film.inv_radius[1] * 16.0f);
                    const uint32_t ix = f2u_sat(pminf(floorf(fx), 15.0f)), iy = f2u_sat(pminf(floorf(fy), 15.0f));
                    const float fw = p.film.table[iy * 16 + ix];
                    const spec c = l * 1.0f * fw;
                    acc.x += c.r; acc.y += c.g; acc.z += c.b; acc.w += fw;
                }
            }
    }
    p.tile_buf[(size_t)lt * slot_px + k] = acc;
}

struct MergeParams {
    FilmRec film;
    int32_t sb[4]; int32_t tile_size, ntx, nty, parts;
    uint32_t slot_w, slot_h;
    const float4* bufs[PH_MAX_TILE_PARTS];
    float* out_xyz; float* out_w;
};
PH_DEV void tile_pixel_bounds(const FilmRec& f, const int tb[4], int pb[4]) {
    const int p0x = f2i_sat(ceilf((float)tb[0] - 0.5f - f.radius[0])), p0y = f2i_sat(ceilf((float)tb[1] - 0.5f - f.radius[1]));
    const int p1x = f2i_sat(floorf((float)tb[2] - 0.5f + f.radius[0])) + 1, p1y = f2i_sat(floorf((float)tb[3] - 0.5f + f.radius[1])) + 1;
    pb[0] = pmaxi(p0x, f.crop[0]); pb[1] = pmaxi(p0y, f.crop[1]); pb[2] = pmini(p1x, f.crop[2]); pb[3] = pmini(p1y, f.crop[3]);
}
__global__ __launch_bounds__(256) void merge_kernel(MergeParams p) {
    const int cw = p.film.crop[2] - p.film.crop[0], ch = p.film.crop[3] - p.film.crop[1];
    const uint64_t gid = (uint64_t)blockIdx.x * blockDim.x + threadIdx.x;
    if (cw <= 0 || ch <= 0 || gid >= (uint64_t)cw * ch) return;
    const int x = p.film.crop[0] + (int)(gid % cw), y = p.film.crop[1] + (int)(gid / cw);
    const int ext_x = (int)ceilf(p.film.radius[0] + 0.5f) + 1, ext_y = (int)ceilf(p.film.radius[1] + 0.5f) + 1;
    const int tx_lo = pmaxi((x - ext_x - p.sb[0]) / p.tile_size - 1, 0), tx_hi = pmini((x + ext_x - p.sb[0]) / p.tile_size + 1, p.ntx - 1);
    const int ty_lo = pmaxi((y - ext_y - p.sb[1]) / p.tile_size - 1, 0), ty_hi = pmini((y + ext_y - p.sb[1]) / p.tile_size + 1, p.nty - 1);
    float X = 0.0f, Y = 0.0f, Z = 0.0f, W = 0.0f;
    const uint32_t slot_px = p.slot_w * p.slot_h;
    for (int ty = ty_lo; ty <= ty_hi; ty++)
        for (int tx = tx_lo; tx <= tx_hi; tx++) {
            int tb[4], pb[4];
            tb[0] = p.sb[0] + tx * p.tile_size; tb[2] = pmini(tb[0] + p.tile_size, p.sb[2]);
            tb[1] = p.sb[1] + ty * p.tile_size; tb[3] = pmini(tb[1] + p.tile_size, p.sb[3]);
            tile_pixel_bounds(p.film, tb, pb);
            if (x < pb[0] || x >= pb[2] || y < pb[1] || y >= pb[3]) continue;
            const uint32_t t = (uint32_t)(ty * p.ntx + tx);
            const float4 c = p.bufs[t % p.parts][(size_t)(t / p.parts) * slot_px + (size_t)(y - pb[1]) * p.slot_w + (size_t)(x - pb[0])];
            X += 0.412453f * c.x + 0.357580f * c.y + 0.180423f * c.z;
            Y += 0.212671f * c.x + 0.715160f * c.y + 0.072169f * c.z;
            Z += 0.019334f * c.x + 0.119193f * c.y + 0.950227f * c.z;
            W += c.w;
        }
    p.out_xyz[3 * gid] = X; p.out_xyz[3 * gid + 1] = Y; p.out_xyz[3 * gid + 2] = Z; p.out_w[gid] = W;
}

__global__ void preset_counters_kernel(IterCounters* ctr, DevStats* stats, uint32_t n) {
    ctr[0].n_cl = n; ctr[0].n_live = n;
    stats->camera_rays += n;
}

__global__ void camera_rays_kernel(DeviceScene sc, CameraRec cam, SamplerRec sp, int x0, int y0, int x1, int y1, uint32_t s, RayIn* out, float* out_pf) {
    const uint32_t gid = blockIdx.x * blockDim.x + threadIdx.x;
    const int wdt = x1 - x0, hgt = y1 - y0;
    if (wdt <= 0 || hgt <= 0 || gid >= (uint32_t)(wdt * hgt)) return;
    const int x = x0 + (int)(gid % wdt), y = y0 + (int)(gid / wdt);
    SamplerCursor c = cursor_for(sc, sp, x, y, s, 0);
    f2 fs = get_2d(sc, sp, c);
    f2 pf = mk2((float)x + fs.x, (float)y + fs.y);
    float tm = get_1d(sc, sp, c);
    f2 lens = get_2d(sc, sp, c);
    RayIn r;
    generate_camera_ray(cam, pf, tm, lens, r);
    store_ray(out + gid, r);
    if (out_pf) { out_pf[2 * gid] = pf.x; out_pf[2 * gid + 1] = pf.y; }
}

}

struct Wavefront {
    std::vector<ph::TileInfo> tiles;
    std::vector<int2> px_xy;
    int sb[4] = {0, 0, 0, 0}, ntx = 0, nty = 0, tile_size = 0, part = 0, parts = 0;
    uint32_t slot_w = 0, slot_h = 0;
    int tiles_key[12] = {0}; bool tiles_valid = false;
    DevBuf d_tiles, d_px, d_rays_cl[2], d_hits, d_rays_sh, d_occ, d_live[2], d_ctr, d_stats, d_cam, d_tex_out;
    DevBuf d_sL, d_sbeta, d_sA, d_sf2, d_sbold, d_sidx, d_sprev, d_recL, d_recpy, d_rounded, d_tilebuf, d_xyz, d_w;
    DevBuf d_vox_slot, d_sp_pool, d_sp_list, d_sp_ctr, d_sp_halton;
    DevBuf d_order, d_sort_bins, d_heads, d_keys_cl, d_keys_sh;
    DevBuf d_morder, d_mkeys, d_mbins;
    size_t n_vox = 0;
    std::vector<hipEvent_t> events;
    phost::ChunkTable chunk_table(bool textured, bool mat_queues) {
        const size_t ray = sizeof(ph::RayIn), hit = sizeof(ph::HitOut);
        return {{&d_rays_cl[0], 2 * ray}, {&d_rays_cl[1], 2 * ray}, {&d_hits, 2 * hit}, {&d_rays_sh, ray}, {&d_occ, 1}, {&d_live[0], 4}, {&d_live[1], 4},
                {&d_sL, 2 * 16}, {&d_sbeta, 2 * 16}, {&d_sA, 2 * 16}, {&d_sf2, 2 * 16}, {&d_sbold, 2 * 16}, {&d_sidx, 2 * 16}, {&d_sprev, 2 * 4},
                {&d_order, 3 * 4}, {&d_keys_cl, 2 * 4}, {&d_keys_sh, 4}, {&d_tex_out, textured ? sizeof(TexOut) : 0, textured}, {&d_morder, 4, mat_queues}, {&d_mkeys, 2, mat_queues}};
    }
    std::vector<DevBuf*> all_bufs() {
        std::vector<DevBuf*> v{&d_tiles, &d_px, &d_ctr, &d_stats, &d_cam, &d_recL, &d_recpy, &d_rounded, &d_tilebuf, &d_xyz, &d_w,
                               &d_vox_slot, &d_sp_pool, &d_sp_list, &d_sp_ctr, &d_sp_halton, &d_sort_bins, &d_heads, &d_mbins};
        for (const phost::ChunkBuf& c : chunk_table(false, false)) v.push_back(c.buf);
        return v;
    }
};

namespace phost {

void free_wavefront(PbrtHipScene* s) {
    Wavefront* w = s->wf;
    if (!w) return;
    for (DevBuf* b : w->all_bufs()) release_buf(*b);
    for (hipEvent_t e : w->events) (void)hipEventDestroy(e);
    delete w;
    s->wf = nullptr;
}

size_t path_chunk_bytes_per_path(bool general, bool textured) { Wavefront w; return chunk_bytes_per_path(w.chunk_table(textured, general || textured)); }
static int sat_i(float v) { if (v != v) return 0; if (v >= 2147483648.0f) return 2147483647; if (v <= -2147483648.0f) return (int)0x80000000; return (int)v; }

struct TileGrid { int sb[4]; int ntx, nty; uint32_t slot_w, slot_h; };
static TileGrid tile_grid(const FilmRec& f, int tile_size) {
    TileGrid g;
    g.sb[0] = sat_i(std::floor((float)f.crop[0] + 0.5f - f.radius[0])); g.sb[1] = sat_i(std::floor((float)f.crop[1] + 0.5f - f.radius[1]));
    g.sb[2] = sat_i(std::ceil((float)f.crop[2] - 0.5f + f.radius[0])); g.sb[3] = sat_i(std::ceil((float)f.crop[3] - 0.5f + f.radius[1]));
    g.ntx = std::max((g.sb[2] - g.sb[0] + tile_size - 1) / tile_size, 0); g.nty = std::max((g.sb[3] - g.sb[1] + tile_size - 1) / tile_size, 0);
    const int e_lo_x = sat_i(std::floor(0.5f + f.radius[0])), e_hi_x = sat_i(std::floor(f.radius[0] - 0.5f)) + 1;
    const int e_lo_y = sat_i(std::floor(0.5f + f.radius[1])), e_hi_y = sat_i(std::floor(f.radius[1] - 0.5f)) + 1;
    g.slot_w = (uint32_t)std::max(tile_size + e_lo_x + e_hi_x, 1); g.slot_h = (uint32_t)std::max(tile_size + e_lo_y + e_hi_y, 1);
    return g;
}

static int setup_tiles(PbrtHipScene* s, int tile_size, int part, int parts) {
    if (!s->wf) s->wf = new Wavefront();
    Wavefront& w = *s->wf;
    const FilmRec& f = s->film;
    const TileGrid g = tile_grid(f, tile_size);
    int key[12] = {f.crop[0], f.crop[1], f.crop[2], f.crop[3], 0, 0, tile_size, part, parts, g.ntx, g.nty, 1};
    std::memcpy(&key[4], &f.radius[0], 4); std::memcpy(&key[5], &f.radius[1], 4);
    if (w.tiles_valid && std::memcmp(key, w.tiles_key, sizeof key) == 0) return PBRT_HIP_OK;
    w.tiles_valid = false;
    const int* sb = g.sb; const int ntx = g.ntx, nty = g.nty;
    w.tiles.clear(); w.px_xy.clear();
    std::memcpy(w.sb, sb, sizeof(w.sb)); w.ntx = ntx; w.nty = nty; w.tile_size = tile_size; w.part = part; w.parts = parts;
    w.slot_w = g.slot_w; w.slot_h = g.slot_h;
    for (int t = part; t < ntx * nty; t += parts) {
        ph::TileInfo ti{};
        const int tx = t % ntx, ty = t / ntx;
        ti.tb[0] = sb[0] + tx * tile_size; ti.tb[2] = std::min(ti.tb[0] + tile_size, sb[2]);
        ti.tb[1] = sb[1] + ty * tile_size; ti.tb[3] = std::min(ti.tb[1] + tile_size, sb[3]);
        const int p0x = sat_i(std::ceil((float)ti.tb[0] - 0.5f - f.radius[0])), p0y = sat_i(std::ceil((float)ti.tb[1] - 0.5f - f.radius[1]));
        const int p1x = sat_i(std::floor((float)ti.tb[2] - 0.5f + f.radius[0])) + 1, p1y = sat_i(std::floor((float)ti.tb[3] - 0.5f + f.radius[1])) + 1;
        ti.pb[0] = std::max(p0x, f.crop[0]); ti.pb[1] = std::max(p0y, f.crop[1]); ti.pb[2] = std::min(p1x, f.crop[2]); ti.pb[3] = std::min(p1y, f.crop[3]);
        ti.px_off = (uint32_t)w.px_xy.size(); ti.tile_index = (uint32_t)t;
        for (int y = ti.tb[1]; y < ti.tb[3]; y++)
            for (int x = ti.tb[0]; x < ti.tb[2]; x++) w.px_xy.push_back(make_int2(x, y));
        w.tiles.push_back(ti);
    }
    int rc;
    if ((rc = ensure_buf(s, w.d_tiles, std::max<size_t>(w.tiles.size(), 1) * sizeof(ph::TileInfo)))) return rc;
// ... 6 lines not shown

size_t tile_buffer_floats_for(const PbrtHipScene* s, int tile_size, int part, int parts) {
    const TileGrid g = tile_grid(s->film, tile_size);
    const int n = g.ntx * g.nty;
    const size_t local = n > part ? (size_t)(n - part + parts - 1) / parts : 0;
    return std::max<size_t>(local, 1) * (size_t)g.slot_w * g.slot_h * 4;
}

static hipEvent_t get_event(PbrtHipScene* s, size_t i) {
    Wavefront& w = *s->wf;
    while (w.events.size() <= i) { hipEvent_t e; if (hipEventCreate(&e) != hipSuccess) return nullptr; w.events.push_back(e); }
    return w.events[i];
}

int check_render_args(PbrtHipScene* s, int max_depth, int light_strategy, const int* pixel_bounds, int tile_size, int part, int parts) {
    if (!s || !pixel_bounds) return set_err(s, PBRT_HIP_ERR_INVALID_ARG, "render: null argument");
    if (!s->built || !s->have_camera || !s->have_film || !s->have_sampler)
        return set_err(s, PBRT_HIP_ERR_STATE, "render: camera, film, sampler and build_accel must be set first");
    if (tile_size <= 0 || parts <= 0 || parts > PH_MAX_TILE_PARTS || part < 0 || part >= parts) return set_err(s, PBRT_HIP_ERR_INVALID_ARG, "render: bad tile partition");
    if (max_depth < 0 || max_depth > 200) return set_err(s, PBRT_HIP_ERR_INVALID_ARG, "render: max_depth out of range");
    if (light_strategy < 0 || light_strategy > 2) return set_err(s, PBRT_HIP_ERR_INVALID_ARG, "render: bad light strategy");
    if (s->sampler.kind == 1 && s->sobol32.empty()) return set_err(s, PBRT_HIP_ERR_STATE, "render: sobol tables not set (pbrt_hip_set_sobol_tables)");
    if (5 + 8 * (max_depth + 1) >= (s->sampler.kind == 0 ? 1000 : 1024)) return set_err(s, PBRT_HIP_ERR_UNSUPPORTED, "render: path would exceed the sampler's dimension table");
    if (s->sampler.kind == 1 && (5 + 8 * (max_depth + 1) > (int)(s->sobol32.size() / 52) || s->sampler.log2_resolution > (int)(s->vdc.size() / 52)))
        return set_err(s, PBRT_HIP_ERR_UNSUPPORTED, "render: path depth or sample-bounds resolution exceeds the Sobol tables given (pbrt_hip_set_sobol_tables)");
    return PBRT_HIP_OK;
}

static int refuse_sphere_lights(PbrtHipScene* s) {
    if (s->sphere_lights == 0) return PBRT_HIP_OK;
    return set_err(s, PBRT_HIP_ERR_UNSUPPORTED, "render: the scene holds a sphere light (pbrt_hip_add_sphere_light), which the path integrator does not sample; render it with pbrt_hip_render_whitted");
}

static int setup_spatial(PbrtHipScene* s, ph::SpatialRec& sr) {
    Wavefront& w = *s->wf;
    const size_t n_lights = s->lights.size();
    float diag[3];
    for (int i = 0; i < 3; i++) { sr.lo[i] = s->bvh.root_lo[i]; sr.hi[i] = s->bvh.root_hi[i]; diag[i] = sr.hi[i] - sr.lo[i]; }
    const int ext = (diag[0] > diag[1] && diag[0] > diag[2]) ? 0 : (diag[1] > diag[2] ? 1 : 2);
    const float bmax = diag[ext];
    size_t nvox = 1;
    for (int i = 0; i < 3; i++) {
        const float r = std::round(diag[i] / bmax * 64.0f);
        long long v = (r != r) ? 0 : (r <= 0.0f ? 0 : (r >= 1048575.0f ? 1048575 : (long long)r));
        sr.nv[i] = (int32_t)std::max<long long>(1, v);
        nvox *= (size_t)sr.nv[i];
    }
    sr.stride = (uint32_t)(2 * n_lights + 2);
    size_t free_b = 0, total_b = 0;
    PH_CHECK(s, hipMemGetInfo(&free_b, &total_b));
    const size_t slot_bytes = (size_t)sr.stride * 4;
    size_t budget = free_b / 2 + w.d_sp_pool.bytes;
    if (const char* e = std::getenv("PBRT_HIP_SPATIAL_POOL_BYTES")) { long long v = std::atoll(e); if (v > 0) budget = (size_t)v; }
    const size_t cap = std::min(nvox, budget / slot_bytes);
    if (cap == 0) return set_err(s, PBRT_HIP_ERR_OOM, "render: no memory for the SpatialLightDistribution pool");
    sr.capacity = (uint32_t)cap;
    int rc;
    if ((rc = ensure_buf(s, w.d_vox_slot, nvox * 4))) return rc;
    w.n_vox = nvox;
    if ((rc = ensure_buf(s, w.d_sp_list, cap * 4))) return rc;
    if ((rc = ensure_buf(s, w.d_sp_ctr, 64))) return rc;
    if ((rc = ensure_buf(s, w.d_sp_pool, cap * slot_bytes))) return rc;
    if (!w.d_sp_halton.p) {
        if ((rc = ensure_buf(s, w.d_sp_halton, 128 * 5 * 4))) return rc;
        static const uint32_t bases[5] = {2, 3, 5, 7, 11};
        float h[128 * 5];
        for (uint64_t i = 0; i < 128; i++)
            for (int d = 0; d < 5; d++) h[5 * i + d] = hm::radical_inverse(bases[d], i);
        PH_CHECK(s, hipMemcpy(w.d_sp_halton.p, h, sizeof h, hipMemcpyHostToDevice));
    }
    PH_CHECK(s, hipMemsetAsync(w.d_vox_slot.p, 0xFF, nvox * 4, s->stream));
    PH_CHECK(s, hipMemsetAsync(w.d_sp_ctr.p, 0, 64, s->stream));
    sr.enabled = 1;
    sr.vox_slot = (int32_t*)w.d_vox_slot.p; sr.pool = (float*)w.d_sp_pool.p; sr.new_list = (uint32_t*)w.d_sp_list.p;
    sr.counters = (uint32_t*)w.d_sp_ctr.p; sr.halton = (const float*)w.d_sp_halton.p;
    return PBRT_HIP_OK;
}

int render_tiles(PbrtHipScene* s, int max_depth, float rr_threshold, int light_strategy, const int pixel_bounds[4], int tile_size, int part,
                        int parts, void* d_tile_buffer, PbrtHipStats* out_stats) {
    int rc;
    PH_CHECK(s, hipSetDevice(s->device));
    if ((rc = upload_scene(s))) return rc;
    const bool spatial = light_strategy == 2 && s->lights.size() > 1;
    if ((rc = upload_light_distribution(s, light_strategy == 2 ? 0 : light_strategy))) return rc;
    if (out_stats) std::memset(out_stats, 0, sizeof(*out_stats));
    SampleRecords rec{};
    if ((rc = samples_begin(s, tile_size, part, parts, &rec))) return rc;
    Wavefront& w = *s->wf;
    const uint32_t spp = s->sampler.spp;
    if (rec.n_px == 0) { PH_CHECK(s, hipMemsetAsync(d_tile_buffer, 0, tile_buffer_floats_for(s, tile_size, part, parts) * 4, s->stream)); PH_CHECK(s, hipStreamSynchronize(s->stream)); return PBRT_HIP_OK; }

    static const ChunkPolicy kChunks{128u << 20, 1u << 20, 0x7FFF0000ull, "render"};
    const bool mat_queues = s->general_materials || s->textured_materials;
    const ChunkTable chunk = w.chunk_table(s->textured_materials, mat_queues);
    if ((rc = samples_plan_bands(s, &rec, chunk_bytes_held(chunk), chunk_bytes_per_path(chunk)))) return rc;
    const uint32_t n_px = rec.band_px;
    const size_t rec_need = (size_t)n_px * spp * 20, rec_have = w.d_recL.bytes + w.d_recpy.bytes;
    uint32_t chunk_spp = plan_chunk_spp_now(kChunks, chunk, rec_need > rec_have ? rec_need - rec_have : 0, n_px, spp);
    const int n_iter = max_depth + 1;
    const int kMaxNullSkips = 1024;
    const int n_iter_cap = s->has_none_material ? n_iter + kMaxNullSkips : n_iter;
    const bool has_quadrics = !s->quadrics.empty();
    if ((rc = ensure_buf(s, w.d_ctr, (size_t)(n_iter_cap + 2) * sizeof(ph::IterCounters)))) return rc;
    if ((rc = ensure_buf(s, w.d_stats, 64 + 6 * PHC_N * 8))) return rc;
    if ((rc = samples_alloc(s, &rec))) return rc;
    if ((rc = chunk_alloc_or_halve(s, kChunks, chunk, n_px, chunk_spp))) return rc;
    const size_t B = (size_t)n_px * chunk_spp;
    chunk_note_footprint(s, B, chunk);

    if ((rc = ensure_traversal_workspace(s))) return rc;
    const uint32_t n_heads = 8, head_chunk = 49152, sort_blocks = 1024;
    ph::RaySortParams sortp{};
    ph::RaySortGrid sort_grid{};
    if ((rc = ensure_buf(s, w.d_sort_bins, 2 * PH_SORT_KEYS * 4))) return rc;
    sortp.order = (uint32_t*)w.d_order.p; sortp.bin_start = (uint32_t*)w.d_sort_bins.p; sortp.bin_cursor = sortp.bin_start + PH_SORT_KEYS;
    sortp.keys_cl = (const uint32_t*)w.d_keys_cl.p; sortp.keys_sh = (const uint32_t*)w.d_keys_sh.p;
    for (int k = 0; k < 3; k++) {
        const float ext = s->bvh.root_hi[k] - s->bvh.root_lo[k];
        sort_grid.lo[k] = s->bvh.root_lo[k]; sort_grid.scale[k] = ext > 0.0f ? 1.0f / ext : 0.0f;
    }
    if ((rc = ensure_buf(s, w.d_heads, (size_t)(n_iter_cap + 2) * n_heads * 64))) return rc;
    ph::MatSortParams msp{};
    if (mat_queues) {
        if ((rc = ensure_buf(s, w.d_mbins, (size_t)(2 * PH_MS_BINS + 1) * 4))) return rc;
        msp.max_depth = max_depth; msp.mat_key = s->ds.mat_key; msp.key_emit = s->ds.ms_key_emit; msp.key_idle = s->ds.ms_key_idle;
        msp.tris = s->ds.tris; msp.meshes = s->ds.meshes; msp.hits = (const ph::HitOut*)w.d_hits.p;
        msp.keys = (uint16_t*)w.d_mkeys.p; msp.order = (uint32_t*)w.d_morder.p;
        msp.bin_start = (uint32_t*)w.d_mbins.p; msp.bin_cursor = msp.bin_start + PH_MS_BINS + 1;
    }

    ph::WfParams wp{};
    wp.cam = s->cam; wp.sp = s->sampler;
    wp.textured = s->textured_materials ? 1u : 0u; wp.cam_dev = nullptr;
    wp.any_rt = 0u;
    for (const MaterialRec& mr : s->materials) if (mr.rt_mode) wp.any_rt = 1u;
    if (s->textured_materials) {
        if ((rc = ensure_buf(s, w.d_cam, sizeof(CameraRec)))) return rc;
        PH_CHECK(s, hipMemcpyAsync(w.d_cam.p, &s->cam, sizeof(CameraRec), hipMemcpyHostToDevice, s->stream));
        wp.cam_dev = (const CameraRec*)w.d_cam.p;
    }
    for (int i = 0; i < 4; i++) wp.pixel_bounds[i] = pixel_bounds[i];
    wp.max_depth = max_depth; wp.rr_threshold = rr_threshold;
    wp.rays_cl[0] = (ph::RayIn*)w.d_rays_cl[0].p; wp.rays_cl[1] = (ph::RayIn*)w.d_rays_cl[1].p;
    wp.hits_cl = (ph::HitOut*)w.d_hits.p; wp.rays_sh = (ph::RayIn*)w.d_rays_sh.p; wp.occ = (uint8_t*)w.d_occ.p;
    wp.live[0] = (uint32_t*)w.d_live[0].p; wp.live[1] = (uint32_t*)w.d_live[1].p;
    wp.ctr = (ph::IterCounters*)w.d_ctr.p; wp.stats = (ph::DevStats*)w.d_stats.p;
    for (int k = 0; k < 2; k++) {
        wp.s_L[k] = (float4*)w.d_sL.p + (size_t)k * B; wp.s_beta[k] = (float4*)w.d_sbeta.p + (size_t)k * B; wp.s_A[k] = (float4*)w.d_sA.p + (size_t)k * B;
        wp.s_f2[k] = (float4*)w.d_sf2.p + (size_t)k * B; wp.s_bold[k] = (float4*)w.d_sbold.p + (size_t)k * B; wp.s_idx[k] = (uint4*)w.d_sidx.p + (size_t)k * B;
        wp.s_prev[k] = (uint32_t*)w.d_sprev.p + (size_t)k * B;
    }
    wp.sort_grid = sort_grid; wp.keys_cl = (uint32_t*)w.d_keys_cl.p; wp.keys_sh = (uint32_t*)w.d_keys_sh.p;
    wp.m_order = mat_queues ? (const uint32_t*)w.d_morder.p : nullptr; wp.m_bins = mat_queues ? (const uint32_t*)w.d_mbins.p : nullptr;

    if (spatial) { if ((rc = setup_spatial(s, wp.spatial))) return rc; }
    PH_CHECK(s, hipMemsetAsync(w.d_stats.p, 0, 64 + 6 * PHC_N * 8, s->stream));
    wp.phase = PH_PHASE_CLOCK ? (unsigned long long*)((char*)w.d_stats.p + 64) : nullptr;
    bool identity = true;
    for (const ph::TileInfo& t : w.tiles)
        if (t.tb[0] < pixel_bounds[0] || t.tb[1] < pixel_bounds[1] || t.tb[2] > pixel_bounds[2] || t.tb[3] > pixel_bounds[3]) { identity = false; break; }
    size_t ev = 0;
    hipEvent_t e_begin = get_event(s, ev++), e_end = get_event(s, ev++);
    if (!e_begin || !e_end) return set_err(s, PBRT_HIP_ERR_DEVICE, "hipEventCreate failed");
    struct Span { hipEvent_t a, b; int kind; };
    std::vector<Span> spans;
// ... 266 lines not shown
}

}

using namespace phost;

extern "C" {

int pbrt_hip_tile_buffer_floats(PbrtHipScene* s, int tile_size, int tile_part, int tile_parts, uint64_t* out_floats) {
    return ph_guard(s, "pbrt_hip_tile_buffer_floats", [&]() -> int {
    if (!s || !out_floats) return PBRT_HIP_ERR_INVALID_ARG;
    if (!s->have_film) return set_err(s, PBRT_HIP_ERR_STATE, "tile_buffer_floats: set_film first");
    if (tile_size <= 0 || tile_parts <= 0 || tile_part < 0 || tile_part >= tile_parts) return set_err(s, PBRT_HIP_ERR_INVALID_ARG, "tile_buffer_floats: bad partition");
    *out_floats = tile_buffer_floats_for(s, tile_size, tile_part, tile_parts);
    return PBRT_HIP_OK;
    });
}

int pbrt_hip_set_sample_record_budget(PbrtHipScene* s, uint64_t bytes) {
    return ph_guard(s, "pbrt_hip_set_sample_record_budget", [&]() -> int {
    if (!s) return PBRT_HIP_ERR_INVALID_ARG;
    s->record_budget = bytes;
    return PBRT_HIP_OK;
    });
}

int pbrt_hip_get_render_footprint(PbrtHipScene* s, uint64_t out[8]) {
    return ph_guard(s, "pbrt_hip_get_render_footprint", [&]() -> int {
    if (!s || !out) return set_err(s, PBRT_HIP_ERR_INVALID_ARG, "get_render_footprint: null argument");
    std::memcpy(out, s->footprint, sizeof s->footprint);
    return PBRT_HIP_OK;
    });
}

int pbrt_hip_render_path_tiles_device(PbrtHipScene* s, int max_depth, float rr_threshold, int light_strategy, const int pixel_bounds[4], int tile_size,
                                      int tile_part, int tile_parts, void* d_tile_buffer, PbrtHipStats* out_stats) {
    return ph_guard(s, "pbrt_hip_render_path_tiles_device", [&]() -> int {
    int rc = check_render_args(s, max_depth, light_strategy, pixel_bounds, tile_size, tile_part, tile_parts);
    if (rc) return rc;
    if ((rc = refuse_sphere_lights(s))) return rc;
    if (!d_tile_buffer) return set_err(s, PBRT_HIP_ERR_INVALID_ARG, "render: null tile buffer");
    return render_tiles(s, max_depth, rr_threshold, light_strategy, pixel_bounds, tile_size, tile_part, tile_parts, d_tile_buffer, out_stats);
    });
}

int pbrt_hip_merge_tiles_device(PbrtHipScene* s, int tile_size, int tile_parts, const void* const* d_tile_buffers, float* out_xyz, float* out_weight) {
    return ph_guard(s, "pbrt_hip_merge_tiles_device", [&]() -> int {
    if (!s || !d_tile_buffers || !out_xyz || !out_weight) return set_err(s, PBRT_HIP_ERR_INVALID_ARG, "merge: null argument");
    if (!s->have_film) return set_err(s, PBRT_HIP_ERR_STATE, "merge: set_film first");
    if (tile_size <= 0 || tile_parts <= 0 || tile_parts > PH_MAX_TILE_PARTS) return set_err(s, PBRT_HIP_ERR_INVALID_ARG, "merge: bad partition");
    PH_CHECK(s, hipSetDevice(s->device));
    return merge_tiles(s, tile_size, tile_parts, d_tile_buffers, out_xyz, out_weight);
    });
}

int pbrt_hip_render_path(PbrtHipScene* s, int max_depth, float rr_threshold, int light_strategy, const int pixel_bounds[4], int tile_size, int tile_part,
                         int tile_parts, float* out_xyz, float* out_weight, PbrtHipStats* out_stats) {
    return ph_guard(s, "pbrt_hip_render_path", [&]() -> int {
    int rc = check_render_args(s, max_depth, light_strategy, pixel_bounds, tile_size, tile_part, tile_parts);
    if (rc) return rc;
    if ((rc = refuse_sphere_lights(s))) return rc;
    if (!out_xyz || !out_weight) return set_err(s, PBRT_HIP_ERR_INVALID_ARG, "render: null output");
    if (s->multi) return render_path_multi(s, max_depth, rr_threshold, light_strategy, pixel_bounds, tile_size, tile_part, tile_parts, out_xyz, out_weight, out_stats);
    DevBuf& tiles = tile_buffer_of(s);
    if ((rc = ensure_buf(s, tiles, tile_buffer_floats_for(s, tile_size, tile_part, tile_parts) * 4))) return rc;
    if ((rc = render_tiles(s, max_depth, rr_threshold, light_strategy, pixel_bounds, tile_size, tile_part, tile_parts, tiles.p, out_stats))) return rc;
    return merge_own_tiles(s, tile_size, tile_part, tile_parts, out_xyz, out_weight);
    });
}

int pbrt_hip_generate_camera_rays(PbrtHipScene* s, const int pb[4], uint32_t sample_index, PbrtHipRay* out_rays, float* out_pfilm) {
    return ph_guard(s, "pbrt_hip_generate_camera_rays", [&]() -> int {
    if (!s || !pb || !out_rays) return set_err(s, PBRT_HIP_ERR_INVALID_ARG, "generate_camera_rays: null argument");
    if (!s->have_camera || !s->have_sampler) return set_err(s, PBRT_HIP_ERR_STATE, "generate_camera_rays: camera and sampler must be set");
    if (s->sampler.kind == 1 && s->sobol32.empty()) return set_err(s, PBRT_HIP_ERR_STATE, "generate_camera_rays: sobol tables not set");
    if (s->sampler.kind == 1 && (s->sobol32.size() / 52 < 5 || s->sampler.log2_resolution > (int)(s->vdc.size() / 52)))
        return set_err(s, PBRT_HIP_ERR_UNSUPPORTED, "generate_camera_rays: sample-bounds resolution exceeds the Sobol tables given");
    PH_CHECK(s, hipSetDevice(s->device));
    const int wdt = pb[2] - pb[0], hgt = pb[3] - pb[1];
    if (wdt <= 0 || hgt <= 0) return PBRT_HIP_OK;
    const size_t n = (size_t)wdt * hgt;
    int rc;
    if ((rc = upload_scene(s))) return rc;
    if ((rc = ensure_buf(s, s->d_rays_tmp, n * sizeof(PbrtHipRay)))) return rc;
    if ((rc = ensure_buf(s, s->d_out_tmp, n * 8))) return rc;
    hipLaunchKernelGGL(ph::camera_rays_kernel, dim3((uint32_t)((n + 255) / 256)), dim3(256), 0, s->stream, s->ds, s->cam, s->sampler, pb[0], pb[1], pb[2], pb[3],
                       sample_index, (ph::RayIn*)s->d_rays_tmp.p, (float*)s->d_out_tmp.p);
    PH_CHECK(s, hipGetLastError());
    PH_CHECK(s, hipMemcpyAsync(out_rays, s->d_rays_tmp.p, n * sizeof(PbrtHipRay), hipMemcpyDeviceToHost, s->stream));
    if (out_pfilm) PH_CHECK(s, hipMemcpyAsync(out_pfilm, s->d_out_tmp.p, n * 8, hipMemcpyDeviceToHost, s->stream));
    PH_CHECK(s, hipStreamSynchronize(s->stream));
    return PBRT_HIP_OK;
    });
}

}

template __global__ void ph::texture_kernel<false, false, 4>(DeviceScene, ph::WfParams, int);
template __global__ void ph::texture_kernel<false, true, 3>(DeviceScene, ph::WfParams, int);
```

### pbrt-v3-rs_amd/csrc/wf_device.h

```cpp
#pragma once
#include "pt_device.h"

namespace ph {

PH_DEV uint32_t wave_alloc(uint32_t* ctr, bool want) {
    const uint64_t m = __ballot(want);
    if (m == 0ull) return 0u;
    const uint32_t lane = threadIdx.x & 63u;
    const int leader = __ffsll((long long)m) - 1;
    uint32_t base = 0;
    if ((int)lane == leader) base = atomicAdd(ctr, (uint32_t)__popcll(m));
    base = __shfl(base, leader);
    const uint64_t lt = (lane == 0) ? 0ull : (~0ull >> (64 - lane));
    return base + (uint32_t)__popcll(m & lt);
}

PH_DEV SamplerCursor cursor_for(const DeviceScene& sc, const SamplerRec& sp, int px, int py, uint32_t s, uint32_t dim, const HaltonLds* lds = nullptr) {
    SamplerCursor c; c.px = px; c.py = py; c.dim = dim; c.lds = lds;
    if (sp.kind == 0) c.index = (uint64_t)halton_pixel_offset(sp, px, py) + (uint64_t)s * sp.sample_stride;
    else c.index = sobol_interval_to_index(sc, (uint32_t)sp.log2_resolution, s, px - sp.bounds[0], py - sp.bounds[1]);
    return c;
}
PH_DEV void store_ray(RayIn* dst, const RayIn& r) {
    float4* p = reinterpret_cast<float4*>(dst);
    p[0] = make_float4(r.ox, r.oy, r.oz, r.t_max); p[1] = make_float4(r.dx, r.dy, r.dz, r.time);
}
PH_DEV RayIn load_ray(const RayIn* src) {
    const float4* p = reinterpret_cast<const float4*>(src);
    float4 a = p[0], b = p[1];
    RayIn r; r.ox = a.x; r.oy = a.y; r.oz = a.z; r.t_max = a.w; r.dx = b.x; r.dy = b.y; r.dz = b.z; r.time = b.w; return r;
}

}
```

### pbrt-v3-rs_amd/csrc/whitted.hip

```cpp
#define PH_OUTLINE_MATH 1
#include "host_math.h"
#include "whitted.h"
#include "scene_host.h"
#include "chunk_plan.h"
#include <algorithm>
#include <cstdlib>
#include <cstring>

struct WhittedWorkspace {
    DevBuf d_rays_cl[2], d_hits, d_rays_sh[2], d_occ, d_live[2], d_ctr, d_stats, d_samples, d_frames;
    phost::ChunkTable chunk_table(uint32_t n_frames) {
        const size_t ray = sizeof(ph::RayIn);
        return {{&d_rays_cl[0], ray}, {&d_rays_cl[1], ray}, {&d_rays_sh[0], PH_WH_SLICE * ray}, {&d_rays_sh[1], PH_WH_SLICE * ray}, {&d_live[0], 4}, {&d_live[1], 4},
                {&d_hits, sizeof(ph::HitOut)}, {&d_occ, PH_WH_SLICE}, {&d_samples, sizeof(ph::WhSample)}, {&d_frames, n_frames * sizeof(ph::WhFrame)}};
    }
    std::vector<DevBuf*> all_bufs() {
        std::vector<DevBuf*> v{&d_ctr, &d_stats};
        for (const phost::ChunkBuf& c : chunk_table(1)) v.push_back(c.buf);
        return v;
    }
};

namespace phost {

void free_whitted(PbrtHipScene* s) {
    WhittedWorkspace* w = s->wh;
    if (!w) return;
    for (DevBuf* b : w->all_bufs()) release_buf(*b);
    delete w;
    s->wh = nullptr;
}

size_t whitted_chunk_bytes_per_sample(uint32_t n_frames) { WhittedWorkspace w; return chunk_bytes_per_path(w.chunk_table(n_frames)); }

static long long whitted_dimension_bound(const PbrtHipScene* s, int max_depth) {
    bool refl = false, trans = false;
    for (const LobeRec& l : s->lobes) if (l.type & ph::BX_SPEC) { refl = refl || (l.type & ph::BX_REFL); trans = trans || (l.type & ph::BX_TRANS); }
    const int d = std::max(max_depth, 1);
    long long vertices = 1, inner = d > 1 ? 1 : 0;
    if (refl && trans) { vertices = (1ll << d) - 1; inner = (1ll << (d - 1)) - 1; }
    else if (refl || trans) { vertices = d; inner = d - 1; }
    return 5 + vertices * 2 * (long long)s->lights.size() + inner * 4;
}

static int check_whitted_args(PbrtHipScene* s, int max_depth, const int* pixel_bounds, int tile_size, int part, int parts) {
    int rc = check_render_args(s, 0, 0, pixel_bounds, tile_size, part, parts);
    if (rc) return rc;
    if (max_depth < 0 || max_depth > PH_WH_MAX_DEPTH) return set_err(s, PBRT_HIP_ERR_INVALID_ARG, "render_whitted: max_depth out of range (0 .. 16)");
    const long long dims = whitted_dimension_bound(s, max_depth);
    if (dims >= (s->sampler.kind == 0 ? 1000 : 1024)) return set_err(s, PBRT_HIP_ERR_UNSUPPORTED, "render_whitted: the recursion could exceed the sampler's dimension table");
    if (s->sampler.kind == 1 && dims > (long long)(s->sobol32.size() / 52))
        return set_err(s, PBRT_HIP_ERR_UNSUPPORTED, "render_whitted: the recursion could draw more dimensions than the Sobol tables given hold (pbrt_hip_set_sobol_tables)");
    return PBRT_HIP_OK;
}

static int render_whitted_tiles(PbrtHipScene* s, int max_depth, const int pixel_bounds[4], int tile_size, int part, int parts, void* d_tile_buffer, PbrtHipStats* out_stats) {
    int rc;
    PH_CHECK(s, hipSetDevice(s->device));
    if ((rc = upload_scene(s))) return rc;
    SampleRecords rec{};
    if ((rc = samples_begin(s, tile_size, part, parts, &rec))) return rc;
    if (out_stats) std::memset(out_stats, 0, sizeof(*out_stats));
    if (rec.n_px == 0) { PH_CHECK(s, hipMemsetAsync(d_tile_buffer, 0, tile_buffer_floats_for(s, tile_size, part, parts) * 4, s->stream)); PH_CHECK(s, hipStreamSynchronize(s->stream)); return PBRT_HIP_OK; }
    if (!s->wh) s->wh = new WhittedWorkspace();
    WhittedWorkspace& w = *s->wh;
    const uint32_t spp = s->sampler.spp, n_frames = (uint32_t)std::max(max_depth, 1);
    const ChunkTable chunk = w.chunk_table(n_frames);
    if ((rc = samples_plan_bands(s, &rec, chunk_bytes_held(chunk), chunk_bytes_per_path(chunk)))) return rc;
    if ((rc = samples_alloc(s, &rec))) return rc;
    const uint32_t n_px = rec.band_px;

    static const ChunkPolicy kChunks{32u << 20, 1u << 16, 0x7FFF0000ull / PH_WH_SLICE, "render_whitted"};
    uint32_t chunk_spp = plan_chunk_spp_now(kChunks, chunk, 0, n_px, spp);
    if ((rc = chunk_alloc_or_halve(s, kChunks, chunk, n_px, chunk_spp))) return rc;
    chunk_note_footprint(s, (size_t)n_px * chunk_spp, chunk);
    if ((rc = ensure_buf(s, w.d_ctr, 2 * sizeof(ph::WhCounters)))) return rc;
    if ((rc = ensure_buf(s, w.d_stats, 64))) return rc;
    if ((rc = ensure_traversal_workspace(s))) return rc;

    ph::WhParams wp{};
    wp.cam = s->cam; wp.sp = s->sampler;
    for (int i = 0; i < 4; i++) wp.pixel_bounds[i] = pixel_bounds[i];
    wp.max_depth = max_depth; wp.n_frames = n_frames;
    wp.diffs = (s->textured_materials || s->bump_materials) ? 1u : 0u;
    for (int k = 0; k < 2; k++) { wp.rays_cl[k] = (ph::RayIn*)w.d_rays_cl[k].p; wp.rays_sh[k] = (ph::RayIn*)w.d_rays_sh[k].p; wp.live[k] = (uint32_t*)w.d_live[k].p; }
    wp.hits_cl = (ph::HitOut*)w.d_hits.p; wp.occ = (uint8_t*)w.d_occ.p;
    wp.ctr = (ph::WhCounters*)w.d_ctr.p; wp.stats = (ph::WhDevStats*)w.d_stats.p;
    wp.samples = (ph::WhSample*)w.d_samples.p; wp.frames = (ph::WhFrame*)w.d_frames.p;
    const bool has_quadrics = !s->quadrics.empty();

    PH_CHECK(s, hipMemsetAsync(w.d_stats.p, 0, 64, s->stream));
    PH_CHECK(s, hipEventRecord(s->ev0, s->stream));
    uint64_t regular = 0, shadow = 0;
    const unsigned long long max_rounds = 1024ull + 1024ull * ((1ull << n_frames) * (2ull + s->lights.size() / PH_WH_SLICE));
    for (size_t band = 0; band < rec.bands.size(); band++) {
        SampleRecords br{};
        if ((rc = samples_band(s, rec, band, &br))) return rc;
        wp.n_px = br.n_px; wp.px_xy = br.px_xy; wp.rec_L = br.rec_L; wp.rec_py = br.rec_py; wp.px_rounded = br.px_rounded;
        for (uint32_t s0 = 0; s0 < spp; s0 += chunk_spp) {
            const uint32_t cs = std::min(chunk_spp, spp - s0);
            wp.chunk_spp = cs; wp.s0 = s0; wp.B = br.n_px * cs;
            const uint32_t blocks = (uint32_t)std::min<size_t>(((size_t)wp.B + 255) / 256, 256 * 16);
            PH_CHECK(s, hipMemsetAsync(w.d_ctr.p, 0, 2 * sizeof(ph::WhCounters), s->stream));
            hipLaunchKernelGGL(ph::whitted_raygen_kernel, dim3((wp.B + 255) / 256), dim3(256), 0, s->stream, s->ds, wp);
            PH_CHECK(s, hipGetLastError());
            for (unsigned long long round = 0;; round++) {
                const int par = (int)(round & 1);
                ph::WhCounters c{};
                PH_CHECK(s, hipMemcpyAsync(&c, wp.ctr + par, sizeof c, hipMemcpyDeviceToHost, s->stream));
                PH_CHECK(s, hipStreamSynchronize(s->stream));
                if (c.n_live == 0) break;
                if (round >= max_rounds) return set_err(s, PBRT_HIP_ERR_UNSUPPORTED, "render_whitted: a sample crossed too many 'none' surfaces");
                regular += c.n_cl; shadow += c.n_sh;
                PH_CHECK(s, hipMemsetAsync(wp.ctr + (par ^ 1), 0, sizeof(ph::WhCounters), s->stream));
                if (c.n_cl || c.n_sh) {
                    ph::TravParams tp{};
                    tp.rays = wp.rays_cl[par]; tp.out = wp.hits_cl; tp.n_ptr = &wp.ctr[par].n_cl; tp.counter = &wp.ctr[par].head;
                    tp.rays2 = wp.rays_sh[par]; tp.out2 = wp.occ; tp.n2_ptr = &wp.ctr[par].n_sh;
                    launch_traverse_kernel(s, 2, std::min<uint32_t>(s->trav_blocks, (c.n_cl + c.n_sh + PH_TRAV_BLOCK - 1) / PH_TRAV_BLOCK), tp);
                    PH_CHECK(s, hipGetLastError());
                }
                if (wp.diffs && c.n_cl) {
                    if (has_quadrics) hipLaunchKernelGGL(ph::whitted_vertex_kernel<true>, dim3(blocks), dim3(PH_TEX_LDS_THREADS), 0, s->stream, s->ds, wp, par);
                    else hipLaunchKernelGGL(ph::whitted_vertex_kernel<false>, dim3(blocks), dim3(PH_TEX_LDS_THREADS), 0, s->stream, s->ds, wp, par);
                    PH_CHECK(s, hipGetLastError());
                }
                if (has_quadrics) hipLaunchKernelGGL(ph::whitted_state_kernel<true>, dim3(blocks), dim3(256), 0, s->stream, s->ds, wp, par);
                else hipLaunchKernelGGL(ph::whitted_state_kernel<false>, dim3(blocks), dim3(256), 0, s->stream, s->ds, wp, par);
                PH_CHECK(s, hipGetLastError());
            }
        }
        if ((rc = samples_to_tiles(s, br, d_tile_buffer))) return rc;
    }
    PH_CHECK(s, hipEventRecord(s->ev1, s->stream));
    PH_CHECK(s, hipStreamSynchronize(s->stream));

    uint32_t flag = 0;
    PH_CHECK(s, hipMemcpy(&flag, s->d_error.p, 4, hipMemcpyDeviceToHost));
    if (flag) { (void)hipMemset(s->d_error.p, 0, 4); return set_err(s, PBRT_HIP_ERR_DEVICE, "traversal stack exceeded 64 entries (the reference panics here, bvh/mod.rs:185)"); }
    if (out_stats) {
        ph::WhDevStats ds;
        PH_CHECK(s, hipMemcpy(&ds, w.d_stats.p, sizeof ds, hipMemcpyDeviceToHost));
// ... 26 lines not shown
```

### pbrt-v3-rs_amd/pbrt_hip/__init__.py

```python
from __future__ import annotations

import ctypes as C
import os
from dataclasses import dataclass

import numpy as np

_HERE = os.path.dirname(os.path.abspath(__file__))
LIB_PATH = os.environ.get("PBRT_HIP_LIB") or os.path.join(os.path.dirname(_HERE), "libpbrt_hip.so")

OK = 0
ERR_INVALID_ARG, ERR_STATE, ERR_DEVICE, ERR_NO_DEVICE, ERR_UNSUPPORTED, ERR_OOM = -1, -2, -3, -4, -5, -6

RAY_DTYPE = np.dtype([("o", "<f4", 3), ("t_max", "<f4"), ("d", "<f4", 3), ("time", "<f4")])
HIT_DTYPE = np.dtype([("t", "<f4"), ("prim", "<u4"), ("b0", "<f4"), ("b1", "<f4"), ("b2", "<f4"), ("pad", "<u4", 3)])
assert RAY_DTYPE.itemsize == 32 and HIT_DTYPE.itemsize == 32


class Stats(C.Structure):
    _fields_ = [
        ("camera_rays", C.c_uint64), ("regular_rays", C.c_uint64), ("shadow_rays", C.c_uint64),
        ("paths_zero_radiance", C.c_uint64), ("paths_total", C.c_uint64),
        ("render_seconds", C.c_double), ("extend_seconds", C.c_double), ("shadow_seconds", C.c_double),
        ("shade_seconds", C.c_double), ("extend_launches", C.c_uint64), ("shadow_launches", C.c_uint64),
# ... 40 lines not shown
            "add_mesh": (C.c_int, [vp, fp, C.c_uint32, u32p, C.c_uint32, fp, fp, fp, C.c_uint32, C.c_int32, C.c_uint32, C.c_float, C.c_float]),
            "add_light_infinite": (C.c_int, [vp, fp, fp, fp]),
            "add_light_distant": (C.c_int, [vp, fp, fp]),
            "add_light_point": (C.c_int, [vp, fp, fp]),
            "add_light_spot": (C.c_int, [vp, fp, fp, fp, C.c_float, C.c_float]),
            "add_light_projection": (C.c_int, [vp, fp, fp, fp, C.c_float, C.c_int, C.c_int, fp]),
            "add_light_goniometric": (C.c_int, [vp, fp, fp, fp, C.c_int, C.c_int, fp]),
            "add_light_diffuse_area": (C.c_int, [vp, fp, C.c_int, C.c_uint32, u32p]),
            "set_camera_perspective": (C.c_int, [vp, fp, fp, C.c_float, C.c_float, C.c_float, C.c_float]),
            "set_camera_orthographic": (C.c_int, [vp, fp, fp, C.c_float, C.c_float, C.c_float, C.c_float]),
            "set_camera_environment": (C.c_int, [vp, fp, C.c_int, C.c_int, C.c_float, C.c_float]),
            "set_film": (C.c_int, [vp, C.c_int, C.c_int, ip, fp, fp, C.c_float, C.c_float]),
            "set_sampler": (C.c_int, [vp, C.c_int, C.c_uint32, ip, C.c_int]),
            "set_sobol_tables": (C.c_int, [vp, u32p, C.c_size_t, C.POINTER(C.c_uint64), C.POINTER(C.c_uint64), C.c_size_t]),
            "build_accel": (C.c_int, [vp, C.c_int, C.c_int]),
            "world_bound": (C.c_int, [vp, fp]),
            "intersect_batch": (C.c_int, [vp, vp, vp, C.c_uint64]),
            "occluded_batch": (C.c_int, [vp, vp, vp, C.c_uint64]),
            "render_path": (C.c_int, [vp, C.c_int, C.c_float, C.c_int, ip, C.c_int, C.c_int, C.c_int, fp, fp, C.POINTER(Stats)]),
            "film_to_rgb": (C.c_int, [vp, fp, fp, fp]),
            "generate_camera_rays": (C.c_int, [vp, ip, C.c_uint32, vp, fp]),
        }
        for name, (res, args) in sig.items():
            fn = f(name)
            fn.restype, fn.argtypes = res, args
        self._optional = {
            "intersect_batch_device": (C.c_int, [vp, vp, vp, C.c_uint64, fp]),
            "occluded_batch_device": (C.c_int, [vp, vp, vp, C.c_uint64, fp]),
            "tile_buffer_floats": (C.c_int, [vp, C.c_int, C.c_int, C.c_int, C.POINTER(C.c_uint64)]),
            "render_whitted": (C.c_int, [vp, C.c_int, ip, C.c_int, C.c_int, C.c_int, fp, fp, C.POINTER(Stats)]),
            "render_path_tiles_device": (C.c_int, [vp, C.c_int, C.c_float, C.c_int, ip, C.c_int, C.c_int, C.c_int, vp, C.POINTER(Stats)]),
            "merge_tiles_device": (C.c_int, [vp, C.c_int, C.c_int, C.POINTER(vp), fp, fp]),
            "add_material_none": (C.c_int, [vp, u32p]),
            "add_material_mirror": (C.c_int, [vp, fp, u32p]),
            "add_material_plastic": (C.c_int, [vp, fp, fp, C.c_float, C.c_int, u32p]),
            "add_material_glass": (C.c_int, [vp, fp, fp, C.c_float, C.c_float, C.c_float, C.c_int, u32p]),
            "add_material_metal": (C.c_int, [vp, fp, fp, C.c_float, C.c_float, C.c_int, u32p]),
            "add_material_uber": (C.c_int, [vp, fp, fp, fp, fp, fp, C.c_float, C.c_float, C.c_float, C.c_int, u32p]),
            "add_material_substrate": (C.c_int, [vp, fp, fp, C.c_float, C.c_float, C.c_int, u32p]),
            "add_material_translucent": (C.c_int, [vp, fp, fp, fp, fp, C.c_float, C.c_int, u32p]),
            "add_material_mix": (C.c_int, [vp, C.c_uint32, C.c_uint32, fp, u32p]),
            "object_begin": (C.c_int, [vp, u32p]),
            "object_end": (C.c_int, [vp]),
            "add_instance": (C.c_int, [vp, C.c_uint32, fp, fp]),
            "add_sphere": (C.c_int, [vp, fp, fp, C.c_float, C.c_float, C.c_float, C.c_float, C.c_uint32, C.c_uint32]),
            "add_sphere_light": (C.c_int, [vp, fp, fp, C.c_float, C.c_float, C.c_float, C.c_float, C.c_uint32, C.c_uint32, fp, C.c_int]),
            "add_hyperboloid": (C.c_int, [vp, fp, fp, fp, fp, C.c_float, C.c_uint32, C.c_uint32]),
            "add_quadric": (C.c_int, [vp, C.c_int, fp, fp, C.c_float, C.c_float, C.c_float, C.c_float, C.c_uint32, C.c_uint32]),
            "add_mipmap": (C.c_int, [vp, C.c_int, C.c_int, fp, C.c_int, C.c_float, C.c_int, C.c_int, C.c_int, C.c_float, u32p]),
            "add_texture_constant": (C.c_int, [vp, fp, u32p]),
            "add_texture_scale": (C.c_int, [vp, C.c_uint32, C.c_uint32, u32p]),
            "add_texture_mix": (C.c_int, [vp, C.c_uint32, C.c_uint32, C.c_uint32, u32p]),
            "add_texture_imagemap": (C.c_int, [vp, C.c_uint32, C.c_float, C.c_float, C.c_float, C.c_float, u32p]),
            "add_texture_checkerboard": (C.c_int, [vp, C.c_uint32, C.c_uint32, C.c_float, C.c_float, C.c_float, C.c_float, C.c_int, u32p]),
            "add_texture_uv": (C.c_int, [vp, C.c_float, C.c_float, C.c_float, C.c_float, u32p]),
            "add_texture_bilerp": (C.c_int, [vp, fp, fp, fp, fp, C.c_float, C.c_float, C.c_float, C.c_float, u32p]),
            "add_texture_dots": (C.c_int, [vp, C.c_uint32, C.c_uint32, C.c_float, C.c_float, C.c_float, C.c_float, u32p]),
            "add_light_infinite_map": (C.c_int, [vp, fp, C.c_int, C.c_int, fp, fp, fp]),
            "add_texture_fbm": (C.c_int, [vp, fp, C.c_float, C.c_int, u32p]),
            "add_texture_wrinkled": (C.c_int, [vp, fp, C.c_float, C.c_int, u32p]),
            "add_texture_windy": (C.c_int, [vp, fp, u32p]),
            "add_texture_marble": (C.c_int, [vp, fp, C.c_float, C.c_int, C.c_float, C.c_float, u32p]),
            "add_texture_checkerboard3d": (C.c_int, [vp, C.c_uint32, C.c_uint32, fp, u32p]),
            "set_texture_mapping": (C.c_int, [vp, C.c_uint32, C.c_int, fp]),
            "add_material_matte_tex": (C.c_int, [vp, C.c_uint32, C.c_float, u32p]),
            "set_material_texture": (C.c_int, [vp, C.c_uint32, C.c_int, C.c_uint32]),
            "set_material_bump": (C.c_int, [vp, C.c_uint32, C.c_uint32]),
            "set_material_float_texture": (C.c_int, [vp, C.c_uint32, C.c_int, C.c_uint32]),
            "set_last_mesh_alpha_textures": (C.c_int, [vp, C.c_uint32, C.c_uint32]),
            "texture_eval_batch": (C.c_int, [vp, C.c_uint32, C.c_uint64, fp, fp]),
            "texture_eval_batch_nodiff": (C.c_int, [vp, C.c_uint32, C.c_uint64, fp, fp]),
            "mipmap_levels": (C.c_int, [vp, C.c_uint32, ip, ip]),
            "mipmap_level_texels": (C.c_int, [vp, C.c_uint32, C.c_int, fp]),
            "set_traversal_counting": (C.c_int, [vp, C.c_int]),
            "get_traversal_counts": (C.c_int, [vp, C.POINTER(C.c_uint64)]),
            "accel_stats": (C.c_int, [vp, C.POINTER(C.c_uint64)]),
            "accel_copy": (C.c_int, [vp, vp, C.c_uint64, vp, C.c_uint64]),
            "build_accel_device": (C.c_int, [vp, C.c_int, C.c_int]),
            "scene_create_multi": (vp, [ip, C.c_int]),
            "scene_devices": (C.c_int, [vp, ip, C.c_int]),
            "selftest_rccl_gather": (C.c_int, [vp, C.c_uint32, C.POINTER(C.c_uint64)]),
            "set_sample_record_budget": (C.c_int, [vp, C.c_uint64]),
            "get_render_footprint": (C.c_int, [vp, C.POINTER(C.c_uint64)]),
        }
        for name, (res, args) in self._optional.items():
            if hasattr(self.lib, prefix + name):
                fn = f(name)
                fn.restype, fn.argtypes = res, args

    def fn(self, name):
        return getattr(self.lib, self.prefix + name)

    def has(self, name):
        return hasattr(self.lib, self.prefix + name)


_default = None


def default_binding() -> Binding:
    global _default
    if _default is None:
        _default = Binding(LIB_PATH, "pbrt_hip_")
    return _default


class Host:

    def __init__(self, binding: Binding | None = None):
        b = binding or default_binding()
        self.lib = b.lib
        fp = C.POINTER(C.c_float)
        L = self.lib
        L.pbrt_hip_host_look_at.restype = C.c_int
        L.pbrt_hip_host_gen_random_tris.argtypes = [C.c_uint64, C.c_uint64, fp, C.POINTER(C.c_uint32)]
        L.pbrt_hip_host_rotate.argtypes = [C.c_float, fp, fp, fp]
        L.pbrt_hip_host_perspective_raster_to_camera.argtypes = [C.c_float, C.c_int, C.c_int, fp, fp]
        L.pbrt_hip_host_orthographic_raster_to_camera.argtypes = [C.c_int, C.c_int, fp, fp]
        L.pbrt_hip_host_transform_points.argtypes = [fp, fp, fp, C.c_size_t]
        L.pbrt_hip_host_transform_vectors.argtypes = [fp, fp, fp, C.c_size_t]
        L.pbrt_hip_host_transform_normals.argtypes = [fp, fp, fp, C.c_size_t]
        ip = C.POINTER(C.c_int)
        L.pbrt_hip_host_film_filter.argtypes = [C.c_int, fp, C.c_int, C.c_int, fp, fp, ip, fp, ip]
        L.pbrt_hip_host_film_filter.restype = C.c_int
        L.pbrt_hip_host_spot.argtypes = [fp, fp, fp, fp, C.c_float, C.c_float, fp, fp, fp]
        L.pbrt_hip_host_swaps_handedness.argtypes = [fp]
        L.pbrt_hip_host_swaps_handedness.restype = C.c_int

    @staticmethod
    def _m():
        return np.zeros(16, np.float32)

    def look_at(self, pos, look, up):
        m, mi = self._m(), self._m()
        rc = self.lib.pbrt_hip_host_look_at(_ptr(_f32(pos), C.c_float), _ptr(_f32(look), C.c_float), _ptr(_f32(up), C.c_float), _ptr(m, C.c_float), _ptr(mi, C.c_float))
        if rc != 0:
            raise PbrtHipError(ERR_INVALID_ARG, "look_at: up vector and viewing direction are parallel")
        return m, mi

    def translate(self, d):
        m, mi = self._m(), self._m()
        self.lib.pbrt_hip_host_translate(_ptr(_f32(d), C.c_float), _ptr(m, C.c_float), _ptr(mi, C.c_float))
        return m, mi

    def scale(self, s):
        m, mi = self._m(), self._m()
        self.lib.pbrt_hip_host_scale(_ptr(_f32(s), C.c_float), _ptr(m, C.c_float), _ptr(mi, C.c_float))
        return m, mi

    def rotate(self, theta_deg, axis):
        m, mi = self._m(), self._m()
        self.lib.pbrt_hip_host_rotate(C.c_float(theta_deg), _ptr(_f32(axis), C.c_float), _ptr(m, C.c_float), _ptr(mi, C.c_float))
        return m, mi

    def compose(self, a, b):
        m, mi = self._m(), self._m()
        self.lib.pbrt_hip_host_compose(_ptr(a[0], C.c_float), _ptr(a[1], C.c_float), _ptr(b[0], C.c_float), _ptr(b[1], C.c_float), _ptr(m, C.c_float), _ptr(mi, C.c_float))
        return m, mi

    def screen_window(self, xres, yres):
        s = np.zeros(4, np.float32)
        self.lib.pbrt_hip_host_screen_window(xres, yres, _ptr(s, C.c_float))
        return s

    def perspective_raster_to_camera(self, fov, xres, yres, screen=None):
        if screen is None:
# ... 408 lines not shown
        for i in range(n.value):
            a = np.zeros((wh[2 * i + 1], wh[2 * i], 3), np.float32)
            self._chk(self.b.fn("mipmap_level_texels")(self.h, mipmap, i, _ptr(a, C.c_float)))
            levels.append(a)
        return levels

    def set_traversal_counting(self, on):
        self._chk(self.b.fn("set_traversal_counting")(self.h, 1 if on else 0))

    def traversal_counts(self):
        c = (C.c_uint64 * 8)()
        self._chk(self.b.fn("get_traversal_counts")(self.h, c))
        return {"closest": {"nodes_passed": int(c[0]), "tri_tests": int(c[1]), "rays": int(c[2]), "ref_node_visits": int(c[2]) + 2 * int(c[0])},
                "any_hit": {"nodes_passed": int(c[3]), "tri_tests": int(c[4]), "rays": int(c[5]), "ref_node_visits": int(c[6])},
                "culled_pops": int(c[7])}

    def devices(self):
        out = np.zeros(64, np.int32)
        n = self.b.fn("scene_devices")(self.h, _ptr(out, C.c_int), 64)
        return [int(v) for v in out[:n]]

    def selftest_rccl_gather(self, n_floats=1 << 20):
        wrong = C.c_uint64(0)
        self._chk(self.b.fn("selftest_rccl_gather")(self.h, n_floats, C.byref(wrong)))
        return int(wrong.value)

    def accel_stats(self):
        c = (C.c_uint64 * 8)()
        self._chk(self.b.fn("accel_stats")(self.h, c))
        return {"interior_nodes": int(c[0]), "leaf_records": int(c[1]), "node_bytes": int(c[2]), "leaf_record_bytes": int(c[3]), "leaves": int(c[4]),
                "depth": int(c[5]), "max_leaf_prims": int(c[6]), "build_seconds": int(c[7]) * 1e-6}

    def accel_copy(self):
        st = self.accel_stats()
        nodes = np.zeros((max(st["interior_nodes"], 1), 16), np.uint32); recs = np.zeros((max(st["leaf_records"], 1), 12), np.uint32)
        self._chk(self.b.fn("accel_copy")(self.h, nodes.ctypes.data, st["interior_nodes"], recs.ctypes.data, st["leaf_records"]))
        return nodes[:st["interior_nodes"]], recs[:st["leaf_records"]]

    def _film_hw(self):
        if self.film_shape is None:
            raise PbrtHipError(ERR_STATE, "set_film must be called before rendering")
        return self.film_shape

    def render_path(self, max_depth=5, rr_threshold=1.0, light_strategy=2, pixel_bounds=None, tile_size=16, tile_part=0, tile_parts=1, out=None):
        h, w = self._film_hw()
        if out is not None:
            xyz, wt = out
            assert xyz.shape == (h, w, 3) and wt.shape == (h, w) and xyz.dtype == np.float32 and wt.dtype == np.float32 and xyz.flags.c_contiguous and wt.flags.c_contiguous
        else:
            xyz = np.zeros((h, w, 3), np.float32); wt = np.zeros((h, w), np.float32)
        pb = np.ascontiguousarray(pixel_bounds if pixel_bounds is not None else self.sample_bounds, dtype=np.int32)
        st = Stats()
        self._chk(self.b.fn("render_path")(self.h, max_depth, C.c_float(rr_threshold), light_strategy, _ptr(pb, C.c_int), tile_size, tile_part, tile_parts,
                                           _ptr(xyz, C.c_float), _ptr(wt, C.c_float), C.byref(st)))
        return xyz, wt, st

    def render_whitted(self, max_depth=5, pixel_bounds=None, tile_size=16, tile_part=0, tile_parts=1):
        h, w = self._film_hw()
        xyz = np.zeros((h, w, 3), np.float32); wt = np.zeros((h, w), np.float32)
        pb = np.ascontiguousarray(pixel_bounds if pixel_bounds is not None else self.sample_bounds, dtype=np.int32)
        st = Stats()
        self._chk(self.b.fn("render_whitted")(self.h, max_depth, _ptr(pb, C.c_int), tile_size, tile_part, tile_parts, _ptr(xyz, C.c_float), _ptr(wt, C.c_float), C.byref(st)))
        return xyz, wt, st

    def set_sample_record_budget(self, nbytes=0):
        self._chk(self.b.fn("set_sample_record_budget")(self.h, int(nbytes)))

    def render_footprint(self):
        c = (C.c_uint64 * 8)()
        self._chk(self.b.fn("get_render_footprint")(self.h, c))
        return {"bands": int(c[0]), "band_tiles": int(c[1]), "record_bytes": int(c[2]), "record_budget": int(c[3]), "chunk_paths": int(c[4]), "chunk_bytes": int(c[5])}

    def film_to_rgb(self, xyz, weight):
        rgb = np.zeros_like(xyz)
        self._chk(self.b.fn("film_to_rgb")(self.h, _ptr(_f32(xyz), C.c_float), _ptr(_f32(weight), C.c_float), _ptr(rgb, C.c_float)))
        return rgb

    def generate_camera_rays(self, pixel_bounds, sample_index):
        pb = np.ascontiguousarray(pixel_bounds, dtype=np.int32)
        n = int((pb[2] - pb[0]) * (pb[3] - pb[1]))
        rays = np.zeros(n, RAY_DTYPE); pf = np.zeros((n, 2), np.float32)
        self._chk(self.b.fn("generate_camera_rays")(self.h, _ptr(pb, C.c_int), sample_index, rays.ctypes.data, _ptr(pf, C.c_float)))
        return rays, pf

    def tile_buffer_floats(self, tile_size, tile_part, tile_parts):
        out = C.c_uint64(0)
        self._chk(self.b.fn("tile_buffer_floats")(self.h, tile_size, tile_part, tile_parts, C.byref(out)))
        return out.value

    def render_path_tiles_device(self, d_tile_buffer_ptr, max_depth=5, rr_threshold=1.0, light_strategy=2, pixel_bounds=None, tile_size=16, tile_part=0, tile_parts=1):
        pb = np.ascontiguousarray(pixel_bounds if pixel_bounds is not None else self.sample_bounds, dtype=np.int32)
        st = Stats()
        self._chk(self.b.fn("render_path_tiles_device")(self.h, max_depth, C.c_float(rr_threshold), light_strategy, _ptr(pb, C.c_int), tile_size, tile_part, tile_parts,
                                                        d_tile_buffer_ptr, C.byref(st)))
        return st

    def merge_tiles_device(self, d_ptrs, tile_size=16, out=None):
        h, w = self._film_hw()
        if out is not None:
            xyz, wt = out
            assert xyz.shape == (h, w, 3) and wt.shape == (h, w) and xyz.dtype == np.float32 and wt.dtype == np.float32 and xyz.flags.c_contiguous and wt.flags.c_contiguous
        else:
            xyz = np.zeros((h, w, 3), np.float32); wt = np.zeros((h, w), np.float32)
        arr = (C.c_void_p * len(d_ptrs))(*d_ptrs)
        self._chk(self.b.fn("merge_tiles_device")(self.h, tile_size, len(d_ptrs), arr, _ptr(xyz, C.c_float), _ptr(wt, C.c_float)))
        return xyz, wt


def read_ply(path):
    with open(path, "rb") as f:
        data = f.read()
    end = data.index(b"end_header") + len(b"end_header")
    end = data.index(b"\n", end) + 1
    header = data[:end].decode("ascii", "replace").split("\n")
    fmt = None; elements = []
    for line in header:
        t = line.split()
        if not t: continue
        if t[0] == "format": fmt = t[1]
        elif t[0] == "element": elements.append({"name": t[1], "n": int(t[2]), "props": []})
        elif t[0] == "property" and elements:
            if t[1] == "list": elements[-1]["props"].append(("list", t[2], t[3], t[4]))
            else: elements[-1]["props"].append(("scalar", t[1], t[2]))
    types = {"char": "i1", "int8": "i1", "uchar": "u1", "uint8": "u1", "short": "i2", "int16": "i2", "ushort": "u2", "uint16": "u2", "int": "i4", "int32": "i4", "uint": "u4", "uint32": "u4",
             "float": "f4", "float32": "f4", "double": "f8", "float64": "f8"}
    P = None; tris = []
    if fmt == "ascii":
        tok = data[end:].split(); pos = 0
        for e in elements:
            if e["name"] == "vertex":
                names = [p[2] for p in e["props"]]; w = len(names)
                a = np.array(tok[pos:pos + w * e["n"]], dtype=np.float64).reshape(e["n"], w); pos += w * e["n"]
                P = np.stack([a[:, names.index(c)] for c in "xyz"], axis=1).astype(np.float32)
            else:
                for _ in range(e["n"]):
                    for pr in e["props"]:
                        if pr[0] == "list":
                            k = int(tok[pos]); v = [int(x) for x in tok[pos + 1:pos + 1 + k]]; pos += 1 + k
                            if e["name"] == "face" and pr[3] in ("vertex_indices", "vertex_index"): tris.append(v)
                        else: pos += 1
    else:
        bo = "<" if fmt == "binary_little_endian" else ">"
        off = end
        for e in elements:
            if all(p[0] == "scalar" for p in e["props"]):
                dt = np.dtype([(p[2], bo + types[p[1]]) for p in e["props"]])
                a = np.frombuffer(data, dt, e["n"], off); off += dt.itemsize * e["n"]
                if e["name"] == "vertex": P = np.stack([a[c] for c in "xyz"], axis=1).astype(np.float32)
            else:
                if e["name"] == "face" and len(e["props"]) == 1:
                    _, ct, it, nm = e["props"][0]; cdt = np.dtype(bo + types[ct]); idt = np.dtype(bo + types[it])
                    done = False
                    for k in (3, 4):
                        rec = np.dtype([("n", cdt), ("v", idt, (k,))])
                        if off + rec.itemsize * e["n"] <= len(data):
                            a = np.frombuffer(data, rec, e["n"], off)
                            if (a["n"] == k).all():
                                if nm in ("vertex_indices", "vertex_index"): tris = a["v"].astype(np.int64)
                                off += rec.itemsize * e["n"]; done = True; break
                    if done: continue
                for _ in range(e["n"]):
                    for pr in e["props"]:
                        if pr[0] == "list":
                            cdt = np.dtype(bo + types[pr[1]]); idt = np.dtype(bo + types[pr[2]])
                            k = int(np.frombuffer(data, cdt, 1, off)[0]); off += cdt.itemsize
                            v = np.frombuffer(data, idt, k, off).astype(np.int64).tolist(); off += idt.itemsize * k
# ... 86 lines not shown
```

Measured before the change: 2332.

## Precompute Halton dimension records and pixel-offset tables, use 32-bit digit reversal

Replaces per-sample Halton work with precomputed per-dimension records (base, 32-bit magic, reciprocal, tail constant) stored in LDS, and a host-built 256-entry pixel-offset table that replaces the per-pixel CRT inverse-radical-inverse loop. Digit reversal now uses a 32-bit mulhi fast path, falling back to a noinline 64-bit path only when the index overflows. The wavefront loop also draws only the sampler dimensions actually needed instead of a fixed 8. It adds a test entry point that compares sampler values, at the cost of extra upload and table-management state.

```diff
diff --git a/include/pbrt_hip.h b/include/pbrt_hip.h
--- a/include/pbrt_hip.h
+++ b/include/pbrt_hip.h
@@ -195,6 +195,8 @@
 
 int pbrt_hip_generate_camera_rays(PbrtHipScene*, const int pixel_bounds[4], uint32_t sample_index,
                                   PbrtHipRay* out_rays, float* out_pfilm_xy);
+int pbrt_hip_sampler_values(PbrtHipScene*, uint32_t n, const int* px, const int* py, const uint32_t* sample, const uint32_t* dim,
+                            float* out);
 
 #ifdef __cplusplus
 }
diff --git a/pbrt-v3-rs_amd/csrc/api.hip b/pbrt-v3-rs_amd/csrc/api.hip
--- a/pbrt-v3-rs_amd/csrc/api.hip
+++ b/pbrt-v3-rs_amd/csrc/api.hip
@@ -54,6 +54,7 @@
     s->owned.clear();
     s->uploaded = false;
     s->light_strategy_uploaded = -1;
+    s->pix_tab_valid = false;
 }
 
 static hm::HaltonTables& halton_tables() {
@@ -87,6 +88,18 @@
             c[k] = PH_LEAF_BIT | t | ((t < n_top && (tris[t].flags & PH_TRI_INSTANCE)) ? PH_LEAF_INST_HINT : 0u);
         }
     nodes[i].c0 = c[0]; nodes[i].c1 = c[1];
+}
+
+__global__ void halton_dims_kernel(HaltonDim* out, const uint32_t* primes, const uint32_t* prime_sums, const uint16_t* perms, uint32_t n) {
+    const uint32_t i = blockIdx.x * blockDim.x + threadIdx.x;
+    if (i >= n) return;
+    const uint32_t base = primes[i];
+    HaltonDim d;
+    d.base = (uint16_t)base; d.perm_at = (uint16_t)prime_sums[i];
+    d.magic = 0xFFFFFFFFu / base;
+    d.inv_base = ph::ph_div(1.0f, (float)base);
+    d.tail = ph::ph_div(d.inv_base * (float)perms[prime_sums[i]], 1.0f - d.inv_base);
+    out[i] = d;
 }
 
 int upload_scene(PbrtHipScene* s) {
@@ -206,7 +219,16 @@
     if ((rc = upload_vec(s, ht.perms, &d.halton_perms))) return rc;
     if ((rc = upload_vec(s, ht.primes, &d.primes))) return rc;
     if ((rc = upload_vec(s, ht.prime_sums, &d.prime_sums))) return rc;
-    if ((rc = upload_vec(s, ht.magic, &d.prime_magic))) return rc;
+    {
+        const uint32_t n_dims = (uint32_t)ht.primes.size();
+        void* dims = nullptr; void* pix = nullptr;
+        PH_CHECK(s, hipMalloc(&dims, n_dims * sizeof(HaltonDim))); s->owned.push_back(dims);
+        PH_CHECK(s, hipMalloc(&pix, PH_HALTON_PIX_TAB * sizeof(uint16_t))); s->owned.push_back(pix);
+        hipLaunchKernelGGL(halton_dims_kernel, dim3((n_dims + 255u) / 256u), dim3(256), 0, s->stream, static_cast<HaltonDim*>(dims), d.primes, d.prime_sums, d.halton_perms, n_dims);
+        PH_CHECK(s, hipGetLastError());
+        d.halton_dims = static_cast<const HaltonDim*>(dims); d.halton_pix = static_cast<const uint16_t*>(pix);
+        s->pix_tab_valid = false;
+    }
     if ((rc = upload_vec(s, s->sobol32, &d.sobol32))) return rc;
     if ((rc = upload_vec(s, s->vdc, &d.vdc))) return rc;
     if ((rc = upload_vec(s, s->vdc_inv, &d.vdc_inv))) return rc;
@@ -219,6 +241,18 @@
     }
     PH_CHECK(s, hipStreamSynchronize(s->stream));
     s->uploaded = true;
+    return PBRT_HIP_OK;
+}
+
+int ensure_sampler_tables(PbrtHipScene* s) {
+    const SamplerRec& r = s->sampler;
+    if (r.kind != 0 || !s->uploaded) return PBRT_HIP_OK;
+    if (s->pix_tab_valid && std::memcmp(&s->pix_tab_for, &r, sizeof(SamplerRec)) == 0) return PBRT_HIP_OK;
+    uint16_t tab[PH_HALTON_PIX_TAB];
+    ph::halton_build_pixel_tables(r, tab);
+    PH_CHECK(s, hipStreamSynchronize(s->stream));
+    PH_CHECK(s, hipMemcpy(const_cast<uint16_t*>(s->ds.halton_pix), tab, sizeof tab, hipMemcpyHostToDevice));
+    s->pix_tab_for = r; s->pix_tab_valid = true;
     return PBRT_HIP_OK;
 }
 
@@ -1253,19 +1287,6 @@
     });
 }
 
-static void ext_gcd(uint64_t a, uint64_t b, int64_t& x, int64_t& y) {
-    if (b == 0) { x = 1; y = 0; return; }
-    int64_t d = (int64_t)(a / b), xp, yp;
-    ext_gcd(b, a % b, xp, yp);
-    x = yp; y = xp - (d * yp);
-}
-static uint64_t mult_inverse(int64_t a, int64_t n) {
-    int64_t x, y;
-    ext_gcd((uint64_t)a, (uint64_t)n, x, y);
-    int64_t r = x - (x / n) * n;
-    return (uint64_t)(r < 0 ? r + n : r);
-}
-
 int pbrt_hip_set_sampler(PbrtHipScene* s, int kind, uint32_t spp, const int sb[4], int at_center) {
     return ph_guard(s, "pbrt_hip_set_sampler", [&]() -> int {
     if (!s || !sb) return set_err(s, PBRT_HIP_ERR_INVALID_ARG, "set_sampler: null argument");
@@ -1276,15 +1297,7 @@
     r.kind = kind; r.spp = spp; r.at_center = at_center ? 1 : 0;
     for (int i = 0; i < 4; i++) r.bounds[i] = sb[i];
     if (kind == 0) {
-        int res[2] = {sb[2] - sb[0], sb[3] - sb[1]};
-        for (int i = 0; i < 2; i++) {
-            uint64_t base = i == 0 ? 2 : 3, scale = 1, e = 0;
-            while ((int)scale < std::min(res[i], 128)) { scale *= base; e++; }
-            r.base_scales[i] = (uint32_t)scale; r.base_exponents[i] = (uint32_t)e;
-        }
-        r.sample_stride = r.base_scales[0] * r.base_scales[1];
-        r.mult_inverse[0] = (uint32_t)mult_inverse(r.base_scales[1], r.base_scales[0]);
-        r.mult_inverse[1] = (uint32_t)mult_inverse(r.base_scales[0], r.base_scales[1]);
+        ph::halton_sampler_setup(r, sb);
         if (((uint64_t)spp + 1) * r.sample_stride >= (1ull << 32))
             return set_err(s, PBRT_HIP_ERR_UNSUPPORTED, "set_sampler: halton index exceeds 32 bits at this spp/resolution");
     } else {
diff --git a/pbrt-v3-rs_amd/csrc/halton_digits.h b/pbrt-v3-rs_amd/csrc/halton_digits.h
--- /dev/null
+++ b/pbrt-v3-rs_amd/csrc/halton_digits.h
@@ -0,0 +1,140 @@
+#pragma once
+#include "scene_types.h"
+#include <stdint.h>
+
+#if defined(__HIPCC__)
+#define PH_HD __host__ __device__ __forceinline__
+#else
+#define PH_HD inline
+#endif
+
+namespace ph {
+
+PH_HD uint32_t hd_mulhi(uint32_t a, uint32_t b) {
+#if defined(__HIP_DEVICE_COMPILE__)
+    return __umulhi(a, b);
+#else
+    return (uint32_t)(((uint64_t)a * b) >> 32);
+#endif
+}
+
+inline void halton_ext_gcd(uint64_t a, uint64_t b, int64_t& x, int64_t& y) {
+    if (b == 0) { x = 1; y = 0; return; }
+    int64_t d = (int64_t)(a / b), xp, yp;
+    halton_ext_gcd(b, a % b, xp, yp);
+    x = yp; y = xp - (d * yp);
+}
+inline uint64_t halton_mult_inverse(int64_t a, int64_t n) {
+    int64_t x, y;
+    halton_ext_gcd((uint64_t)a, (uint64_t)n, x, y);
+    int64_t r = x - (x / n) * n;
+    return (uint64_t)(r < 0 ? r + n : r);
+}
+inline void halton_sampler_setup(SamplerRec& r, const int sb[4]) {
+    const int res[2] = {sb[2] - sb[0], sb[3] - sb[1]};
+    for (int i = 0; i < 2; i++) {
+        uint64_t base = i == 0 ? 2 : 3, scale = 1, e = 0;
+        while ((int)scale < (res[i] < 128 ? res[i] : 128)) { scale *= base; e++; }
+        r.base_scales[i] = (uint32_t)scale; r.base_exponents[i] = (uint32_t)e;
+    }
+    r.sample_stride = r.base_scales[0] * r.base_scales[1];
+    r.mult_inverse[0] = (uint32_t)halton_mult_inverse(r.base_scales[1], r.base_scales[0]);
+    r.mult_inverse[1] = (uint32_t)halton_mult_inverse(r.base_scales[0], r.base_scales[1]);
+}
+
+PH_HD uint32_t inverse_radical_inverse(uint32_t base, uint32_t inverse, uint32_t n_digits) {
+    uint32_t index = 0;
+    for (uint32_t i = 0; i < n_digits; i++) { uint32_t digit = inverse % base; inverse /= base; index = index * base + digit; }
+    return index;
+}
+PH_HD int rem_i(int a, int b) { int r = a - (a / b) * b; return r < 0 ? r + b : r; }
+
+PH_HD uint32_t halton_pixel_offset_crt(const SamplerRec& sp, int px, int py) {
+    uint64_t off = 0;
+    if (sp.sample_stride > 1) {
+        const int pm[2] = {rem_i(px, 128), rem_i(py, 128)};
+        for (int i = 0; i < 2; i++) {
+            uint64_t dim_offset = inverse_radical_inverse(i == 0 ? 2u : 3u, (uint32_t)pm[i], sp.base_exponents[i]);
+            off += dim_offset * (uint64_t)(sp.sample_stride / sp.base_scales[i]) * (uint64_t)sp.mult_inverse[i];
+        }
+        off %= sp.sample_stride;
+    }
+    return (uint32_t)off;
+}
+#define PH_HALTON_PIX_TAB 256
+inline void halton_build_pixel_tables(const SamplerRec& sp, uint16_t tab[PH_HALTON_PIX_TAB]) {
+    for (int i = 0; i < 2; i++)
+        for (uint32_t r = 0; r < 128; r++) {
+            uint64_t t = 0;
+            if (sp.sample_stride > 1) {
+                const uint64_t dim_offset = inverse_radical_inverse(i == 0 ? 2u : 3u, r, sp.base_exponents[i]);
+                t = dim_offset * (uint64_t)(sp.sample_stride / sp.base_scales[i]) * (uint64_t)sp.mult_inverse[i] % sp.sample_stride;
+            }
+            tab[128 * i + r] = (uint16_t)t;
+        }
+}
+PH_HD uint32_t halton_pixel_offset(const SamplerRec& sp, const uint16_t* __restrict__ tab, int px, int py) {
+    uint32_t off = (uint32_t)tab[(uint32_t)px & 127u] + (uint32_t)tab[128u + ((uint32_t)py & 127u)];
+    if (off >= sp.sample_stride) off -= sp.sample_stride;
+    return off;
+}
+
+PH_HD void halton_divmod(uint32_t a, uint32_t base, uint32_t magic, uint32_t& q, uint32_t& r) {
+    q = hd_mulhi(a, magic);
+    r = a - q * base;
+    if (r >= base) { q += 1u; r -= base; }
+}
+PH_HD void halton_divmod_small(uint32_t a, uint32_t base, uint32_t magic, uint32_t& q, uint32_t& r) {
+    q = hd_mulhi(a, magic + 1u);
+    r = a - q * base;
+}
+PH_HD bool halton_fits_32(uint32_t a, uint32_t base) { return hd_mulhi(a, base) == 0u; }
+
+template <typename PermT>
+PH_HD uint32_t halton_reverse_32(uint32_t a, uint32_t base, uint32_t magic, const PermT* __restrict__ perm, float inv_base, float& inv_base_n) {
+    uint32_t reversed = 0;
+    while (a != 0) {
+        uint32_t next, digit;
+        halton_divmod_small(a, base, magic, next, digit);
+        reversed = reversed * base + (uint32_t)perm[digit];
+        inv_base_n *= inv_base;
+        a = next;
+    }
+    return reversed;
+}
+template <typename PermT>
+PH_HD uint64_t halton_reverse_64(uint32_t a, uint32_t base, uint32_t magic, const PermT* __restrict__ perm, float inv_base, float& inv_base_n) {
+    uint64_t reversed = 0;
+    while (a != 0) {
+        uint32_t next, digit;
+        halton_divmod(a, base, magic, next, digit);
+        reversed = reversed * base + (uint64_t)perm[digit];
+        inv_base_n *= inv_base;
+        a = next;
+    }
+    return reversed;
+}
+PH_HD uint32_t halton_reverse3_32(uint32_t a, float inv_base, float& inv_base_n) {
+    uint32_t reversed = 0;
+    while (a != 0) {
+        uint32_t next, digit;
+        halton_divmod_small(a, 3u, 0x55555555u, next, digit);
+        reversed = reversed * 3u + digit;
+        inv_base_n *= inv_base;
+        a = next;
+    }
+    return reversed;
+}
+PH_HD uint64_t halton_reverse3_64(uint32_t a, float inv_base, float& inv_base_n) {
+    uint64_t reversed = 0;
+    while (a != 0) {
+        uint32_t next, digit;
+        halton_divmod(a, 3u, 0x55555555u, next, digit);
+        reversed = reversed * 3u + digit;
+        inv_base_n *= inv_base;
+        a = next;
+    }
+    return reversed;
+}
+
+}
diff --git a/pbrt-v3-rs_amd/csrc/host_math.h b/pbrt-v3-rs_amd/csrc/host_math.h
--- a/pbrt-v3-rs_amd/csrc/host_math.h
+++ b/pbrt-v3-rs_amd/csrc/host_math.h
@@ -69,7 +69,6 @@
 struct HaltonTables {
     std::vector<uint32_t> primes, prime_sums;
     std::vector<uint16_t> perms;
-    std::vector<uint64_t> magic;
     void build() {
         primes.clear(); prime_sums.clear();
         for (uint32_t c = 2; primes.size() < 1000; c++) {
@@ -78,8 +77,7 @@
             if (is_p) primes.push_back(c);
         }
         uint32_t total = 0;
-        magic.clear();
-        for (uint32_t p : primes) { prime_sums.push_back(total); total += p; magic.push_back((uint64_t)(((unsigned __int128)1 << 64) / p) + 1); }
+        for (uint32_t p : primes) { prime_sums.push_back(total); total += p; }
         perms.assign(total, 0);
         Pcg32 rng; size_t at = 0;
         for (uint32_t p : primes) {
diff --git a/pbrt-v3-rs_amd/csrc/pt_device.h b/pbrt-v3-rs_amd/csrc/pt_device.h
--- a/pbrt-v3-rs_amd/csrc/pt_device.h
+++ b/pbrt-v3-rs_amd/csrc/pt_device.h
@@ -1,6 +1,7 @@
 #pragma once
 #include "dmath.h"
 #include "scene_types.h"
+#include "halton_digits.h"
 #include "traverse.h"
 
 namespace ph {
@@ -12,81 +13,47 @@
     uint64_t r = ((uint64_t)__brev((uint32_t)a) << 32) | (uint64_t)__brev((uint32_t)(a >> 32));
     return __ull2float_rn(r) * 0x1.0p-64f;
 }
-PH_DEV float radical_inverse_base(uint32_t base, uint32_t a) {
-    const float inv_base = ph_div(1.0f, (float)base);
-    uint64_t reversed = 0;
+PH_DEV float radical_inverse_3(uint32_t a) {
+    const float inv_base = ph_div(1.0f, 3.0f);
     float inv_base_n = 1.0f;
-    while (a != 0) {
-        uint32_t next = a / base, digit = a - next * base;
-        reversed = reversed * base + digit;
-        inv_base_n *= inv_base;
-        a = next;
-    }
+    if (halton_fits_32(a, 3u)) { const uint32_t reversed = halton_reverse3_32(a, inv_base, inv_base_n); return pminf(__uint2float_rn(reversed) * inv_base_n, kOneMinusEps); }
+    const uint64_t reversed = halton_reverse3_64(a, inv_base, inv_base_n);
     return pminf(__ull2float_rn(reversed) * inv_base_n, kOneMinusEps);
 }
-PH_DEV float scrambled_radical_inverse(uint32_t base, uint64_t magic, uint32_t a, const uint16_t* __restrict__ perm) {
-    const float inv_base = ph_div(1.0f, (float)base);
-    uint64_t reversed = 0;
+__device__ __noinline__ float scrambled_radical_inverse_wide(const HaltonDim* d, uint32_t a, const void* perm, bool perm_bytes) {
     float inv_base_n = 1.0f;
-    while (a != 0) {
-        uint32_t next = (uint32_t)__umul64hi((uint64_t)a, magic), digit = a - next * base;
-        reversed = reversed * base + perm[digit];
-        inv_base_n *= inv_base;
-        a = next;
-    }
-    return pminf(inv_base_n * (__ull2float_rn(reversed) + ph_div(inv_base * (float)perm[0], 1.0f - inv_base)), kOneMinusEps);
-}
-PH_DEV uint32_t inverse_radical_inverse(uint32_t base, uint32_t inverse, uint32_t n_digits) {
-    uint32_t index = 0;
-    for (uint32_t i = 0; i < n_digits; i++) { uint32_t digit = inverse % base; inverse /= base; index = index * base + digit; }
-    return index;
-}
-PH_DEV int rem_i(int a, int b) { int r = a - (a / b) * b; return r < 0 ? r + b : r; }
-
-PH_DEV uint32_t halton_pixel_offset(const SamplerRec& sp, int px, int py) {
-    uint64_t off = 0;
-    if (sp.sample_stride > 1) {
-        const int pm[2] = {rem_i(px, 128), rem_i(py, 128)};
-        for (int i = 0; i < 2; i++) {
-            uint64_t dim_offset = inverse_radical_inverse(i == 0 ? 2u : 3u, (uint32_t)pm[i], sp.base_exponents[i]);
-            off += dim_offset * (uint64_t)(sp.sample_stride / sp.base_scales[i]) * (uint64_t)sp.mult_inverse[i];
-        }
-        off %= sp.sample_stride;
-    }
-    return (uint32_t)off;
+    const uint64_t reversed = perm_bytes ? halton_reverse_64(a, d->base, d->magic, static_cast<const uint8_t*>(perm), d->inv_base, inv_base_n)
+                                         : halton_reverse_64(a, d->base, d->magic, static_cast<const uint16_t*>(perm), d->inv_base, inv_base_n);
+    return pminf(inv_base_n * (__ull2float_rn(reversed) + d->tail), kOneMinusEps);
+}
+template <typename PermT>
+PH_DEV float scrambled_radical_inverse(const HaltonDim* d, uint32_t a, const PermT* __restrict__ perm) {
+    const uint32_t base = d->base;
+    if (!halton_fits_32(a, base)) return scrambled_radical_inverse_wide(d, a, perm, sizeof(PermT) == 1);
+    const float inv_base = d->inv_base;
+    float inv_base_n = 1.0f;
+    const uint32_t reversed = halton_reverse_32(a, base, d->magic, perm, inv_base, inv_base_n);
+    return pminf(inv_base_n * (__uint2float_rn(reversed) + d->tail), kOneMinusEps);
 }
 #define PH_LDS_DIMS 54
 #define PH_LDS_PERMS 6081
 struct HaltonLds {
-    uint8_t perms[PH_LDS_PERMS + 2];
-    uint32_t primes[PH_LDS_DIMS], sums[PH_LDS_DIMS];
-    uint64_t magic[PH_LDS_DIMS];
+    HaltonDim dims[PH_LDS_DIMS];
+    uint8_t perms[PH_LDS_PERMS + 7];
 };
 PH_DEV void halton_lds_fill(HaltonLds* l, const DeviceScene& sc) {
     for (uint32_t i = threadIdx.x; i < PH_LDS_PERMS; i += blockDim.x) l->perms[i] = (uint8_t)sc.halton_perms[i];
-    for (uint32_t i = threadIdx.x; i < PH_LDS_DIMS; i += blockDim.x) { l->primes[i] = sc.primes[i]; l->sums[i] = sc.prime_sums[i]; l->magic[i] = sc.prime_magic[i]; }
-}
-PH_DEV float scrambled_radical_inverse_lds(const HaltonLds* l, uint32_t dim, uint32_t a) {
-    const uint32_t base = l->primes[dim];
-    const uint64_t magic = l->magic[dim];
-    const uint8_t* perm = l->perms + l->sums[dim];
-    const float inv_base = ph_div(1.0f, (float)base);
-    uint64_t reversed = 0;
-    float inv_base_n = 1.0f;
-    while (a != 0) {
-        uint32_t next = (uint32_t)__umul64hi((uint64_t)a, magic), digit = a - next * base;
-        reversed = reversed * base + perm[digit];
-        inv_base_n *= inv_base;
-        a = next;
-    }
-    return pminf(inv_base_n * (__ull2float_rn(reversed) + ph_div(inv_base * (float)perm[0], 1.0f - inv_base)), kOneMinusEps);
+    for (uint32_t i = threadIdx.x; i < PH_LDS_DIMS; i += blockDim.x) l->dims[i] = sc.halton_dims[i];
+}
+PH_DEV float halton_sample_scrambled(const DeviceScene& sc, uint32_t index, uint32_t dim, const HaltonLds* lds) {
+    if (lds && dim < PH_LDS_DIMS) { const HaltonDim* d = lds->dims + dim; return scrambled_radical_inverse(d, index, lds->perms + d->perm_at); }
+    return scrambled_radical_inverse(sc.halton_dims + dim, index, sc.halton_perms + sc.prime_sums[dim]);
 }
 PH_DEV float halton_sample(const DeviceScene& sc, const SamplerRec& sp, uint32_t index, uint32_t dim, const HaltonLds* lds = nullptr) {
     if (sp.at_center && (dim == 0 || dim == 1)) return 0.5f;
     if (dim == 0) return radical_inverse_2((uint64_t)(index >> sp.base_exponents[0]));
-    if (dim == 1) return radical_inverse_base(3u, index / sp.base_scales[1]);
-    if (lds && dim < PH_LDS_DIMS) return scrambled_radical_inverse_lds(lds, dim, index);
-    return scrambled_radical_inverse(sc.primes[dim], sc.prime_magic[dim], index, sc.halton_perms + sc.prime_sums[dim]);
+    if (dim == 1) return radical_inverse_3(index / sp.base_scales[1]);
+    return halton_sample_scrambled(sc, index, dim, lds);
 }
 
 PH_DEV uint64_t sobol_interval_to_index(const DeviceScene& sc, uint32_t m, uint64_t frame, int px, int py) {
@@ -121,6 +88,9 @@
 };
 PH_DEV float sampler_dim(const DeviceScene& sc, const SamplerRec& sp, const SamplerCursor& c, uint32_t dim) {
     return sp.kind == 0 ? halton_sample(sc, sp, (uint32_t)c.index, dim, c.lds) : sobol_sample(sc, sp, c.index, dim, c.px, c.py);
+}
+PH_DEV float sampler_dim_scrambled(const DeviceScene& sc, const SamplerRec& sp, const SamplerCursor& c, uint32_t dim) {
+    return sp.kind == 0 ? halton_sample_scrambled(sc, (uint32_t)c.index, dim, c.lds) : sobol_sample(sc, sp, c.index, dim, c.px, c.py);
 }
 PH_DEV float get_1d(const DeviceScene& sc, const SamplerRec& sp, SamplerCursor& c) {
     float p = sampler_dim(sc, sp, c, c.dim);
diff --git a/pbrt-v3-rs_amd/csrc/scene_host.h b/pbrt-v3-rs_amd/csrc/scene_host.h
--- a/pbrt-v3-rs_amd/csrc/scene_host.h
+++ b/pbrt-v3-rs_amd/csrc/scene_host.h
@@ -77,6 +77,7 @@
     bool uploaded = false;
     int light_strategy_uploaded = -1;
     DevBuf d_ld_func, d_ld_cdf;
+    SamplerRec pix_tab_for{}; bool pix_tab_valid = false;
 
     DevBuf d_counter, d_spill, d_error, d_rays_tmp, d_out_tmp;
     uint32_t trav_blocks = 0;
@@ -99,6 +100,7 @@
 void projection_light_setup(float fov_deg, float aspect, float out_proj[16], float out_screen[4], float* out_cos_total_width);
 void hmip_lookup_triangle(const PbrtHipScene* s, const MipRec& m, float u, float v, float width, float out[3]);
 int upload_light_distribution(PbrtHipScene* s, int light_strategy);
+int ensure_sampler_tables(PbrtHipScene* s);
 int launch_traverse(PbrtHipScene* s, bool anyhit, const void* d_rays, void* d_out, uint32_t n, float* kernel_ms);
 void launch_traverse_kernel(PbrtHipScene* s, int mode, uint32_t blocks, const ph::TravParams& p);
 int ensure_traversal_workspace(PbrtHipScene* s);
diff --git a/pbrt-v3-rs_amd/csrc/scene_types.h b/pbrt-v3-rs_amd/csrc/scene_types.h
--- a/pbrt-v3-rs_amd/csrc/scene_types.h
+++ b/pbrt-v3-rs_amd/csrc/scene_types.h
@@ -191,6 +191,12 @@
     uint32_t base_scales[2], base_exponents[2], sample_stride;
     uint32_t mult_inverse[2];
     int32_t resolution, log2_resolution;
+};
+
+struct alignas(16) HaltonDim {
+    uint32_t magic;
+    float inv_base, tail;
+    uint16_t base, perm_at;
 };
 
 struct DeviceScene {
@@ -232,7 +238,8 @@
     const uint16_t* halton_perms;
     const uint32_t* primes;
     const uint32_t* prime_sums;
-    const uint64_t* prime_magic;
+    const HaltonDim* halton_dims;
+    const uint16_t* halton_pix;
     const uint32_t* sobol32;
     const uint64_t* vdc;
     const uint64_t* vdc_inv;
diff --git a/pbrt-v3-rs_amd/csrc/wavefront.hip b/pbrt-v3-rs_amd/csrc/wavefront.hip
--- a/pbrt-v3-rs_amd/csrc/wavefront.hip
+++ b/pbrt-v3-rs_amd/csrc/wavefront.hip
@@ -377,8 +377,9 @@
                         PHC_END(2);
                         PHC_BEGIN(3);
                         SamplerCursor cur = cursor_for(sc, w.sp, xy.x, xy.y, w.s0 + (pid - ppix * w.chunk_spp), dim, hl);
+                        const uint32_t n_draw = (sc.n_lights > 0 ? 7u : 2u) + (__ballot(bounces > 3u) != 0ull ? 1u : 0u);
 #pragma unroll 1
-                        for (uint32_t k = 0; k < 8; k++) s_u[k][tid] = sampler_dim(sc, w.sp, cur, dim + k);
+                        for (uint32_t k = 0; k < n_draw; k++) s_u[k][tid] = TEX ? sampler_dim_scrambled(sc, w.sp, cur, dim + k) : sampler_dim(sc, w.sp, cur, dim + k);
                         PHC_END(3);
                         uint32_t c = 0;
                         if (BO::has_non_specular(bsdf)) {
@@ -682,6 +683,19 @@
     if (out_pf) { out_pf[2 * gid] = pf.x; out_pf[2 * gid + 1] = pf.y; }
 }
 
+__global__ __launch_bounds__(256) void sampler_values_kernel(DeviceScene sc, SamplerRec sp, uint32_t n, const int* px, const int* py, const uint32_t* sample, const uint32_t* dims, float* out) {
+    __shared__ HaltonLds halton_lds;
+    const HaltonLds* hl = nullptr;
+    if (sp.kind == 0) { halton_lds_fill(&halton_lds, sc); hl = &halton_lds; }
+    __syncthreads();
+    const uint32_t i = blockIdx.x * blockDim.x + threadIdx.x;
+    if (i >= n) return;
+    const SamplerCursor c0 = cursor_for(sc, sp, px[i], py[i], sample[i], dims[i]);
+    const SamplerCursor c1 = cursor_for(sc, sp, px[i], py[i], sample[i], dims[i], hl);
+    out[i] = sampler_dim(sc, sp, c0, dims[i]);
+    out[n + i] = sampler_dim(sc, sp, c1, dims[i]);
+}
+
 }
 
 struct Wavefront {
@@ -854,6 +868,7 @@
     int rc;
     PH_CHECK(s, hipSetDevice(s->device));
     if ((rc = upload_scene(s))) return rc;
+    if ((rc = ensure_sampler_tables(s))) return rc;
     const bool spatial = light_strategy == 2 && s->lights.size() > 1;
     if ((rc = upload_light_distribution(s, light_strategy == 2 ? 0 : light_strategy))) return rc;
     if (out_stats) std::memset(out_stats, 0, sizeof(*out_stats));
@@ -1286,6 +1301,7 @@
     const size_t n = (size_t)wdt * hgt;
     int rc;
     if ((rc = upload_scene(s))) return rc;
+    if ((rc = ensure_sampler_tables(s))) return rc;
     if ((rc = ensure_buf(s, s->d_rays_tmp, n * sizeof(PbrtHipRay)))) return rc;
     if ((rc = ensure_buf(s, s->d_out_tmp, n * 8))) return rc;
     hipLaunchKernelGGL(ph::camera_rays_kernel, dim3((uint32_t)((n + 255) / 256)), dim3(256), 0, s->stream, s->ds, s->cam, s->sampler, pb[0], pb[1], pb[2], pb[3],
@@ -1298,6 +1314,38 @@
     });
 }
 
+int pbrt_hip_sampler_values(PbrtHipScene* s, uint32_t n, const int* px, const int* py, const uint32_t* sample, const uint32_t* dim, float* out) {
+    return ph_guard(s, "pbrt_hip_sampler_values", [&]() -> int {
+    if (!s || !px || !py || !sample || !dim || !out) return set_err(s, PBRT_HIP_ERR_INVALID_ARG, "sampler_values: null argument");
+    if (!s->have_sampler) return set_err(s, PBRT_HIP_ERR_STATE, "sampler_values: the sampler must be set");
+    if (n == 0) return PBRT_HIP_OK;
+    const uint32_t dim_limit = s->sampler.kind == 0 ? 1000u : (uint32_t)(s->sobol32.size() / 52);
+    if (s->sampler.kind == 1 && s->sampler.log2_resolution > (int)(s->vdc.size() / 52)) return set_err(s, PBRT_HIP_ERR_UNSUPPORTED, "sampler_values: sample-bounds resolution exceeds the Sobol tables given");
+    for (uint32_t i = 0; i < n; i++) {
+        if (dim[i] >= dim_limit) return set_err(s, PBRT_HIP_ERR_INVALID_ARG, "sampler_values: dimension outside the sampler's tables");
+        if (s->sampler.kind == 0 && (uint64_t)sample[i] > s->sampler.spp) return set_err(s, PBRT_HIP_ERR_INVALID_ARG, "sampler_values: sample index above spp");
+    }
+    PH_CHECK(s, hipSetDevice(s->device));
+    int rc;
+    if ((rc = upload_scene(s))) return rc;
+    if ((rc = ensure_sampler_tables(s))) return rc;
+    const size_t nb = (size_t)n * 4;
+    if ((rc = ensure_buf(s, s->d_rays_tmp, 4 * nb))) return rc;
+    if ((rc = ensure_buf(s, s->d_out_tmp, 2 * nb))) return rc;
+    char* in = (char*)s->d_rays_tmp.p;
+    PH_CHECK(s, hipMemcpyAsync(in, px, nb, hipMemcpyHostToDevice, s->stream));
+    PH_CHECK(s, hipMemcpyAsync(in + nb, py, nb, hipMemcpyHostToDevice, s->stream));
+    PH_CHECK(s, hipMemcpyAsync(in + 2 * nb, sample, nb, hipMemcpyHostToDevice, s->stream));
+    PH_CHECK(s, hipMemcpyAsync(in + 3 * nb, dim, nb, hipMemcpyHostToDevice, s->stream));
+    hipLaunchKernelGGL(ph::sampler_values_kernel, dim3((n + 255u) / 256u), dim3(256), 0, s->stream, s->ds, s->sampler, n, (const int*)in, (const int*)(in + nb),
+                       (const uint32_t*)(in + 2 * nb), (const uint32_t*)(in + 3 * nb), (float*)s->d_out_tmp.p);
+    PH_CHECK(s, hipGetLastError());
+    PH_CHECK(s, hipMemcpyAsync(out, s->d_out_tmp.p, 2 * nb, hipMemcpyDeviceToHost, s->stream));
+    PH_CHECK(s, hipStreamSynchronize(s->stream));
+    return PBRT_HIP_OK;
+    });
+}
+
 }
 
 template __global__ void ph::texture_kernel<false, false, 4>(DeviceScene, ph::WfParams, int);
diff --git a/pbrt-v3-rs_amd/csrc/wf_device.h b/pbrt-v3-rs_amd/csrc/wf_device.h
--- a/pbrt-v3-rs_amd/csrc/wf_device.h
+++ b/pbrt-v3-rs_amd/csrc/wf_device.h
@@ -17,7 +17,7 @@
 
 PH_DEV SamplerCursor cursor_for(const DeviceScene& sc, const SamplerRec& sp, int px, int py, uint32_t s, uint32_t dim, const HaltonLds* lds = nullptr) {
     SamplerCursor c; c.px = px; c.py = py; c.dim = dim; c.lds = lds;
-    if (sp.kind == 0) c.index = (uint64_t)halton_pixel_offset(sp, px, py) + (uint64_t)s * sp.sample_stride;
+    if (sp.kind == 0) c.index = (uint64_t)halton_pixel_offset(sp, sc.halton_pix, px, py) + (uint64_t)s * sp.sample_stride;
     else c.index = sobol_interval_to_index(sc, (uint32_t)sp.log2_resolution, s, px - sp.bounds[0], py - sp.bounds[1]);
     return c;
 }
diff --git a/pbrt-v3-rs_amd/csrc/whitted.hip b/pbrt-v3-rs_amd/csrc/whitted.hip
--- a/pbrt-v3-rs_amd/csrc/whitted.hip
+++ b/pbrt-v3-rs_amd/csrc/whitted.hip
@@ -58,6 +58,7 @@
     int rc;
     PH_CHECK(s, hipSetDevice(s->device));
     if ((rc = upload_scene(s))) return rc;
+    if ((rc = ensure_sampler_tables(s))) return rc;
     SampleRecords rec{};
     if ((rc = samples_begin(s, tile_size, part, parts, &rec))) return rc;
     if (out_stats) std::memset(out_stats, 0, sizeof(*out_stats));
diff --git a/pbrt-v3-rs_amd/pbrt_hip/__init__.py b/pbrt-v3-rs_amd/pbrt_hip/__init__.py
--- a/pbrt-v3-rs_amd/pbrt_hip/__init__.py
+++ b/pbrt-v3-rs_amd/pbrt_hip/__init__.py
@@ -146,6 +146,7 @@
             "selftest_rccl_gather": (C.c_int, [vp, C.c_uint32, C.POINTER(C.c_uint64)]),
             "set_sample_record_budget": (C.c_int, [vp, C.c_uint64]),
             "get_render_footprint": (C.c_int, [vp, C.POINTER(C.c_uint64)]),
+            "sampler_values": (C.c_int, [vp, C.c_uint32, ip, ip, u32p, u32p, fp]),
         }
         for name, (res, args) in self._optional.items():
             if hasattr(self.lib, prefix + name):
@@ -720,6 +721,15 @@
         rays = np.zeros(n, RAY_DTYPE); pf = np.zeros((n, 2), np.float32)
         self._chk(self.b.fn("generate_camera_rays")(self.h, _ptr(pb, C.c_int), sample_index, rays.ctypes.data, _ptr(pf, C.c_float)))
         return rays, pf
+
+    def sampler_values(self, px, py, sample, dim):
+        px = np.ascontiguousarray(px, dtype=np.int32); py = np.ascontiguousarray(py, dtype=np.int32)
+        sample = np.ascontiguousarray(sample, dtype=np.uint32); dim = np.ascontiguousarray(dim, dtype=np.uint32)
+        n = len(px)
+        assert len(py) == n and len(sample) == n and len(dim) == n
+        out = np.zeros(2 * n, np.float32)
+        self._chk(self.b.fn("sampler_values")(self.h, n, _ptr(px, C.c_int), _ptr(py, C.c_int), _ptr(sample, C.c_uint32), _ptr(dim, C.c_uint32), _ptr(out, C.c_float)))
+        return out[:n], out[n:]
 
     def tile_buffer_floats(self, tile_size, tile_part, tile_parts):
         out = C.c_uint64(0)
```

New measurement: 2352 (median of 6 runs). Within noise of the previous version (+0.8%).
